# ibm-granite/dolomite-engine

Measured on AMD Instinct MI355X. Metric: tokens/sec/node GPTDolomite-3B bf16 seq4096 padding-free, higher is better.
Workload: dtype bf16; 1 GPU; gptdolomite-3b-bf16-seq4096-paddingfree-pretrain; model=GPTDolomite-3B, global_batch=16, seq_len=4096, parallelism=dp1

## Files before the change

### dolomite_engine_amd/csrc/attention.hip

```cpp

#include "common.h"

typedef __bf16 bf16x8 __attribute__((ext_vector_type(8)));
typedef float f32x4 __attribute__((ext_vector_type(4)));
typedef uint32_t u32x4 __attribute__((ext_vector_type(4)));

#define MFMA16(a, b, c) __builtin_amdgcn_mfma_f32_16x16x32_bf16((a), (b), (c), 0, 0, 0)

#define DOL_LOG2E 1.44269504088896340736f
#define DOL_LN2 0.69314718055994530942f

#define PI23(q) (((q) & ~12) | ((((q) >> 2) & 1) << 3) | ((((q) >> 3) & 1) << 2))

typedef __bf16 bf16x4 __attribute__((ext_vector_type(4)));


__device__ __forceinline__ bf16x8 lds_tr16_bfrag(const __bf16* img, int rowbase, int S, int d0, int lane) {
    const int g8 = (lane >> 4) * 8;
    const int jj = (lane >> 2) & 3;
    const int cc = (lane & 3) * 4;
    unsigned a0 = (unsigned)(size_t)(img + PI23(rowbase + g8 + jj) * S + d0 + cc);
    unsigned a1 = (unsigned)(size_t)(img + PI23(rowbase + g8 + 4 + jj) * S + d0 + cc);
    bf16x4 lo, hi;
    asm volatile(
        "ds_read_b64_tr_b16 %0, %2\n\t"
        "ds_read_b64_tr_b16 %1, %3\n\t"
        "s_waitcnt lgkmcnt(0)"
        : "=&v"(lo), "=&v"(hi)
        : "v"(a0), "v"(a1)
        : "memory");
    bf16x8 out;
#pragma unroll
    for (int t = 0; t < 4; ++t) { out[t] = lo[t]; out[4 + t] = hi[t]; }
    return out;
}


template <int OFF>
__device__ __forceinline__ void tr16_issue(unsigned a0, unsigned a1, bf16x4& lo, bf16x4& hi) {
    asm volatile(
        "ds_read_b64_tr_b16 %0, %2 offset:%c4\n\t"
        "ds_read_b64_tr_b16 %1, %3 offset:%c4"
        : "=&v"(lo), "=&v"(hi)
        : "v"(a0), "v"(a1), "i"(OFF)
        : "memory");
}

template <int N>
__device__ __forceinline__ void lgkm_wait2(bf16x4& a, bf16x4& b) {
    asm volatile("s_waitcnt lgkmcnt(%c2)" : "+v"(a), "+v"(b) : "i"(N));
}
template <int N>
__device__ __forceinline__ void lgkm_wait4(bf16x4& a, bf16x4& b, bf16x4& c, bf16x4& d) {
    asm volatile("s_waitcnt lgkmcnt(%c4)" : "+v"(a), "+v"(b), "+v"(c), "+v"(d) : "i"(N));
}
template <int N>
__device__ __forceinline__ void lgkm_wait8(bf16x4& a, bf16x4& b, bf16x4& c, bf16x4& d,
                                           bf16x4& e, bf16x4& f, bf16x4& g, bf16x4& h) {
    asm volatile("s_waitcnt lgkmcnt(%c8)"
                 : "+v"(a), "+v"(b), "+v"(c), "+v"(d), "+v"(e), "+v"(f), "+v"(g), "+v"(h)
                 : "i"(N));
}

__device__ __forceinline__ bf16x8 tr16_join8(bf16x4 lo, bf16x4 hi) {
    bf16x8 out;
#pragma unroll
    for (int t = 0; t < 4; ++t) { out[t] = lo[t]; out[4 + t] = hi[t]; }
    return out;
}

__device__ __forceinline__ bf16x8 load_bf16x8_guard(const __bf16* p, int d0, int D, bool valid) {
    const __bf16* q = (d0 < D) ? p : (p - d0);
    bool ok = valid && (d0 < D);
    bf16x8 r = *(const bf16x8*)q;
#pragma unroll
    for (int e = 0; e < 8; ++e) r[e] = ok ? r[e] : (__bf16)0.f;
    return r;
}

__device__ __forceinline__ void xcd_remap_tile_bh(int& tile, int& b, int& h) {
    const int ntile = gridDim.x, nb = gridDim.y, nh = gridDim.z;
    const int64_t nbh = (int64_t)nb * nh;
    if (nbh % 8 != 0) return;
    int64_t raw = blockIdx.x + (int64_t)ntile * (blockIdx.y + (int64_t)nb * blockIdx.z);
    int xcd = (int)(raw % 8);
    int64_t idx = raw / 8;
    int64_t pair_local = idx / ntile;
    tile = (int)(idx % ntile);
    int64_t pair = pair_local * 8 + xcd;
    b = (int)(pair % nb);
    h = (int)(pair / nb);
}

#define DOL_DROP_CQ 0x9E3779B1u
#define DOL_DROP_CK 0x85EBCA77u
#define DOL_DROP_CH 0xC2B2AE3Du
#define DOL_DROP_M1 0x7FEB352Du
#define DOL_DROP_M2 0x846CA68Bu

__device__ __forceinline__ uint32_t drop_mix32(uint32_t x) {
    x ^= x >> 16;
    x *= DOL_DROP_M1;
    x ^= x >> 15;
    x *= DOL_DROP_M2;
    x ^= x >> 16;
    return x;
}
__device__ __forceinline__ uint32_t drop_head_word(uint32_t seed_hi, uint32_t h) {
    return drop_mix32(seed_hi ^ (h * DOL_DROP_CH));
}
__device__ __forceinline__ uint32_t drop_row_word(uint32_t seed_lo, uint32_t t_q) {
    return drop_mix32(seed_lo ^ (t_q * DOL_DROP_CQ));
}
__device__ __forceinline__ uint32_t drop_col_word(uint32_t head_word, uint32_t t_k) {
    return drop_mix32(head_word ^ (t_k * DOL_DROP_CK));
}
__device__ __forceinline__ bool drop_keep_words(uint32_t rw, uint32_t cw, uint32_t thr) {
    uint32_t x = rw ^ cw;
    x ^= x >> 16;
    x *= DOL_DROP_M1;
    x ^= x >> 15;
    x *= DOL_DROP_M2;
    return x >= thr;
}
__device__ __forceinline__ bool drop_keep(uint32_t seed_lo, uint32_t seed_hi, uint32_t h,
                                          uint32_t t_q, uint32_t t_k, uint32_t thr) {
    return drop_keep_words(drop_row_word(seed_lo, t_q),
                           drop_col_word(drop_head_word(seed_hi, h), t_k), thr);
}

static inline uint32_t drop_threshold(float p_drop) {
    return (uint32_t)((double)p_drop * 4294967296.0);
}
static inline bool drop_p_valid(float p_drop) { return p_drop >= 0.f && p_drop < 1.f; }


template <int DPAD>
struct FaKvLds {
    static constexpr int S = DPAD + 16;
    static constexpr size_t image_bytes = (size_t)2 * 64 * S * sizeof(__bf16);
    static constexpr size_t bytes(bool dropout) {
        return image_bytes + (dropout ? 64 * sizeof(uint32_t) : 0);
    }
};

__device__ __forceinline__ void fa_tr16_perm_bases(const __bf16* img, int S, int lane,
                                                   unsigned& a0, unsigned& a1) {
    const int row = (lane >> 4) * 4 + ((lane >> 2) & 3);
    const int cc = (lane & 3) * 4;
    a0 = (unsigned)(size_t)(img + row * S + cc);
    a1 = (unsigned)(size_t)(img + (16 + row) * S + cc);
}

__device__ __forceinline__ float qgroup_reduce_max(float v) {
    auto a = __builtin_amdgcn_permlane16_swap(__float_as_uint(v), __float_as_uint(v), false, false);
    v = fmaxf(__uint_as_float(a[0]), __uint_as_float(a[1]));
    auto b = __builtin_amdgcn_permlane32_swap(__float_as_uint(v), __float_as_uint(v), false, false);
    return fmaxf(__uint_as_float(b[0]), __uint_as_float(b[1]));
}
__device__ __forceinline__ float qgroup_reduce_sum(float v) {
    auto a = __builtin_amdgcn_permlane16_swap(__float_as_uint(v), __float_as_uint(v), false, false);
    v = __uint_as_float(a[0]) + __uint_as_float(a[1]);
    auto b = __builtin_amdgcn_permlane32_swap(__float_as_uint(v), __float_as_uint(v), false, false);
    return __uint_as_float(b[0]) + __uint_as_float(b[1]);
}


template <int DPAD, bool DROPOUT>
__global__ void __launch_bounds__(512, 4) fa_fwd_kernel(
    const __bf16* __restrict__ q, const __bf16* __restrict__ k, const __bf16* __restrict__ v,
    __bf16* __restrict__ o, float* __restrict__ lse,
    const int32_t* __restrict__ seq_begin, const int32_t* __restrict__ seq_end,
    int H, int Hkv, int D, int G,
    int64_t q_ts, int64_t q_gs, int64_t k_ts, int64_t k_hs, int64_t v_ts, int64_t v_hs,
    int64_t o_ts, int64_t T_total, float scale,
    uint32_t seed_lo, uint32_t seed_hi, uint32_t drop_thr, float drop_rp) {
    constexpr int KCH = DPAD / 32;
    constexpr int DCH = DPAD / 16;
    constexpr int SK = FaKvLds<DPAD>::S;

    int tile_id = blockIdx.x, b = blockIdx.y, h = blockIdx.z;
    xcd_remap_tile_bh(tile_id, b, h);
    const int s0 = __builtin_amdgcn_readfirstlane(seq_begin[b]);
    const int L = __builtin_amdgcn_readfirstlane(seq_end[b]) - s0;
    const int ntile_seq = (L + 127) / 128;
    if (tile_id >= ntile_seq) return;
    const int qs = (ntile_seq - 1 - tile_id) * 128;

    const int lane = threadIdx.x & 63;
    const int wave = threadIdx.x >> 6;
    const int lr = lane & 15;
    const int lg = lane >> 4;

    extern __shared__ char smem_raw[];
    __bf16* Klds = (__bf16*)smem_raw;
    __bf16* Vlds = Klds + 64 * SK;
    uint32_t* Cw = (uint32_t*)(Vlds + 64 * SK);

    const int kvh = h / G;
    const int64_t q_hoff = (int64_t)(h / G) * q_gs + (int64_t)(h % G) * D;

    const int qrow = qs + wave * 16 + lr;
    const bool qvalid = qrow < L;
    bf16x8 qf[KCH];
#pragma unroll
    for (int kc = 0; kc < KCH; ++kc) {
        int d0 = kc * 32 + lg * 8;
        const __bf16* p = q + (int64_t)(s0 + (qvalid ? qrow : 0)) * q_ts + q_hoff + d0;
        qf[kc] = load_bf16x8_guard(p, d0, D, qvalid);
    }

    float m_run = -INFINITY, l_run = 0.f;
    f32x4 o_acc[DCH];
#pragma unroll
    for (int dc = 0; dc < DCH; ++dc) o_acc[dc] = {0.f, 0.f, 0.f, 0.f};

    uint32_t drop_rw = 0;
    uint32_t drop_hw = 0;
    if constexpr (DROPOUT) {
        drop_hw = drop_head_word(seed_hi, (uint32_t)h);
        drop_rw = drop_row_word(seed_lo, (uint32_t)(s0 + qrow));
    }

    unsigned aV0, aV1;
    fa_tr16_perm_bases(Vlds, SK, lane, aV0, aV1);

    const int kend = min(L, qs + 128);
    const int ntiles = (kend + 63) / 64;

    if (D < DPAD) {
        for (int pidx = threadIdx.x; pidx < 64 * (DPAD - D) / 8; pidx += 512) {
            int key = pidx / ((DPAD - D) / 8);
            int d0 = D + (pidx % ((DPAD - D) / 8)) * 8;
            bf16x8 z = {};
            *(bf16x8*)&Klds[key * SK + d0] = z;
            *(bf16x8*)&Vlds[key * SK + d0] = z;
        }
    }

    int st_koff[2], st_voff[2];
    int st_klds[2], st_vlds[2];
#pragma unroll
    for (int j = 0; j < 2; ++j) {
        int pidx = (int)threadIdx.x + j * 512;
        int pp = pidx < 64 * D / 8 ? pidx : 0;
        int key = pp / (D / 8);
        int d0 = (pp % (D / 8)) * 8;
        st_koff[j] = (int)(key * k_ts + kvh * k_hs) + d0;
        st_voff[j] = (int)(key * v_ts + kvh * v_hs) + d0;
        st_klds[j] = key * SK + d0;
        st_vlds[j] = key * SK + d0;
    }

    if (__builtin_amdgcn_readfirstlane(threadIdx.x) >= 256) __builtin_amdgcn_s_setprio(1);

    constexpr int PIECES = 64 * DPAD / 8;

    auto stage_direct = [&](int ks_, __bf16* Kw, __bf16* Vw) {
        if (ks_ + 64 <= kend) {
            const int64_t disp = (int64_t)(s0 + ks_);
#pragma unroll
            for (int j = 0; j < 2; ++j) {
                if ((int)threadIdx.x + j * 512 < 64 * D / 8) {
                    *(bf16x8*)&Kw[st_klds[j]] = *(const bf16x8*)(k + disp * k_ts + st_koff[j]);
                    *(bf16x8*)&Vw[st_vlds[j]] = *(const bf16x8*)(v + disp * v_ts + st_voff[j]);
                }
            }
        } else {
            for (int pidx = threadIdx.x; pidx < PIECES; pidx += 512) {
                int key = pidx / (DPAD / 8);
                int d0 = (pidx % (DPAD / 8)) * 8;
                bool kv_valid = (ks_ + key) < kend;
                const __bf16* kp = k + (int64_t)(s0 + (kv_valid ? ks_ + key : 0)) * k_ts + (int64_t)kvh * k_hs + d0;
                *(bf16x8*)&Kw[key * SK + d0] = load_bf16x8_guard(kp, d0, D, kv_valid);
                const __bf16* vp = v + (int64_t)(s0 + (kv_valid ? ks_ + key : 0)) * v_ts + (int64_t)kvh * v_hs + d0;
                *(bf16x8*)&Vw[key * SK + d0] = load_bf16x8_guard(vp, d0, D, kv_valid);
            }
        }
    };

    const float scale2 = scale * DOL_LOG2E;

    auto compute_tile = [&](const __bf16* Kb, unsigned aV0c, unsigned aV1c, int ks) {
        f32x4 sc[4];
#pragma unroll
        for (int cb = 0; cb < 4; ++cb) {
            sc[cb] = {0.f, 0.f, 0.f, 0.f};
#pragma unroll
            for (int kc = 0; kc < KCH; ++kc) {
                bf16x8 kf = *(const bf16x8*)&Kb[(cb * 16 + lr) * SK + kc * 32 + lg * 8];
                sc[cb] = MFMA16(kf, qf[kc], sc[cb]);
            }
        }

        const bool edge_tile =
            !((ks + 63 <= qs + wave * 16) && (ks + 64 <= kend) && (qs + wave * 16 + 16 <= L));
        if (__builtin_amdgcn_readfirstlane(edge_tile ? 1 : 0)) {
#pragma unroll
            for (int cb = 0; cb < 4; ++cb) {
#pragma unroll
                for (int x = 0; x < 4; ++x) {
                    const int kpos = ks + cb * 16 + lg * 4 + x;
                    if (kpos > qrow || kpos >= kend || qrow >= L) sc[cb][x] = -INFINITY;
                }
            }
        }
        float mx[4];
#pragma unroll
        for (int cb = 0; cb < 4; ++cb)
            mx[cb] = fmaxf(fmaxf(sc[cb][0], sc[cb][1]), fmaxf(sc[cb][2], sc[cb][3]));
        const float rowmax = qgroup_reduce_max(fmaxf(fmaxf(mx[0], mx[1]), fmaxf(mx[2], mx[3])));
        float mnew = fmaxf(m_run, rowmax * scale2);
        if (mnew == -INFINITY) mnew = 0.f;
        const float alpha = exp2f(m_run - mnew);
        m_run = mnew;

        bf16x8 pf[2];
        float rsum = 0.f;
#pragma unroll
        for (int cb = 0; cb < 4; ++cb) {
            u32x4 cw = {};
            if constexpr (DROPOUT) cw = *(const u32x4*)&Cw[cb * 16 + lg * 4];
#pragma unroll
            for (int x = 0; x < 4; ++x) {
                const float e = exp2f(fmaf(sc[cb][x], scale2, -mnew));
                float ek = e;
                if constexpr (DROPOUT) ek = drop_keep_words(drop_rw, cw[x], drop_thr) ? e : 0.f;
                pf[cb >> 1][(cb & 1) * 4 + x] = (__bf16)ek;
                rsum += e;
            }
        }
        l_run = l_run * alpha + rsum;
        if (!__all(alpha == 1.0f)) {
#pragma unroll
            for (int dc = 0; dc < DCH; ++dc) o_acc[dc] *= alpha;
        }

        {
            __builtin_amdgcn_sched_barrier(0);
            bf16x4 vlo[3], vhi[3];
            tr16_issue<0>(aV0c, aV1c, vlo[0], vhi[0]);
            tr16_issue<((1 / DCH) * 32 * SK + (1 % DCH) * 16) * 2>(aV0c, aV1c, vlo[1], vhi[1]);
#define FWD_PV_STEP(i)                                                                                  \
    if constexpr ((i) < 2 * DCH) {                                                                      \
        constexpr int kc2_ = (i) / DCH, dc_ = (i) % DCH;                                                \
        if constexpr ((i) + 2 < 2 * DCH) {                                                              \
            constexpr int kn_ = ((i) + 2) / DCH, dn_ = ((i) + 2) % DCH;                                 \
            tr16_issue<(kn_ * 32 * SK + dn_ * 16) * 2>(aV0c, aV1c, vlo[((i) + 2) % 3], vhi[((i) + 2) % 3]); \
            lgkm_wait2<4>(vlo[(i) % 3], vhi[(i) % 3]);                                                  \
        } else if constexpr ((i) + 1 < 2 * DCH) {                                                       \
            lgkm_wait2<2>(vlo[(i) % 3], vhi[(i) % 3]);                                                  \
        } else {                                                                                        \
            lgkm_wait2<0>(vlo[(i) % 3], vhi[(i) % 3]);                                                  \
        }                                                                                               \
        o_acc[dc_] = MFMA16(tr16_join8(vlo[(i) % 3], vhi[(i) % 3]), pf[kc2_], o_acc[dc_]);              \
    }
            FWD_PV_STEP(0) FWD_PV_STEP(1) FWD_PV_STEP(2) FWD_PV_STEP(3)
            FWD_PV_STEP(4) FWD_PV_STEP(5) FWD_PV_STEP(6) FWD_PV_STEP(7)
            FWD_PV_STEP(8) FWD_PV_STEP(9) FWD_PV_STEP(10) FWD_PV_STEP(11)
            FWD_PV_STEP(12) FWD_PV_STEP(13) FWD_PV_STEP(14) FWD_PV_STEP(15)
#undef FWD_PV_STEP
            __builtin_amdgcn_sched_barrier(0);
        }
    };

    for (int kt = 0; kt < ntiles; ++kt) {
        stage_direct(kt * 64, Klds, Vlds);
        if constexpr (DROPOUT) {
            if (__builtin_amdgcn_readfirstlane(threadIdx.x) < 64)
                Cw[lane] = drop_col_word(drop_hw, (uint32_t)(s0 + kt * 64 + lane));
        }
        __syncthreads();
        compute_tile(Klds, aV0, aV1, kt * 64);
        __syncthreads();
    }

    const float l_row = qgroup_reduce_sum(l_run);
    float inv_l = (l_row > 0.f) ? 1.f / l_row : 0.f;
    if constexpr (DROPOUT) inv_l *= drop_rp;
    if (lg == 0 && qvalid)
        lse[(int64_t)h * T_total + s0 + qrow] = (m_run + log2f(l_row)) * DOL_LN2;
    __bf16* orow = o + (int64_t)(s0 + (qvalid ? qrow : 0)) * o_ts + (int64_t)h * D;
#pragma unroll
    for (int dc = 0; dc < DCH; ++dc) {
        const int d0 = dc * 16 + lg * 4;
        bf16x4 ov;
#pragma unroll
        for (int x = 0; x < 4; ++x) ov[x] = (__bf16)(o_acc[dc][x] * inv_l);
        if (qvalid && d0 < D) *(bf16x4*)&orow[d0] = ov;
    }
}

struct FaProblem {
    dolomite_stream_t stream;
    const void *q, *k, *v;
    void* o;
    const void* dout;
    float* lse;
    const float* delta;
    void* dqkv_q;
    float *dk_acc, *dv_acc;
    const int32_t *seq_begin, *seq_end;
    int batch, max_seqlen;
    int64_t T;
    int H, Hkv, D, G;
    int64_t q_ts, q_gs, k_ts, k_hs, v_ts, v_hs, do_ts;
    float scale;
    int dtype;
    float p_drop;
    uint64_t seed;
    bool gaps;
};

static int fa_check_args(const FaProblem& p, bool fwd) {
    if (!drop_p_valid(p.p_drop)) return 9013;
    if (p.dtype != DOLOMITE_BF16) return 9010;
    if (p.D > 128) return 9011;
    if (fwd && !(p.scale > 0.f)) return 9015;
    return 0;
}

template <typename Launch>
static int fa_select_kernel(const FaProblem& p, Launch launch) {
    auto by_dpad = [&](auto drop) {
        if (p.D <= 32) return launch(std::integral_constant<int, 32>{}, drop);
        if (p.D <= 64) return launch(std::integral_constant<int, 64>{}, drop);
        if (p.D <= 96) return launch(std::integral_constant<int, 96>{}, drop);
        return launch(std::integral_constant<int, 128>{}, drop);
    };
    return p.p_drop > 0.f ? by_dpad(std::true_type{}) : by_dpad(std::false_type{});
}

static dim3 fa_grid(const FaProblem& p) { return dim3((p.max_seqlen + 127) / 128, p.batch, p.H); }

template <int DPAD, bool DROPOUT>
static int launch_fa_fwd(const FaProblem& p) {
    hipLaunchKernelGGL((fa_fwd_kernel<DPAD, DROPOUT>), fa_grid(p), dim3(512), FaKvLds<DPAD>::bytes(DROPOUT),
                       (hipStream_t)p.stream, (const __bf16*)p.q, (const __bf16*)p.k, (const __bf16*)p.v,
                       (__bf16*)p.o, p.lse, p.seq_begin, p.seq_end, p.H, p.Hkv, p.D, p.G,
                       p.q_ts, p.q_gs, p.k_ts, p.k_hs, p.v_ts, p.v_hs, (int64_t)p.H * p.D, p.T, p.scale,
                       (uint32_t)p.seed, (uint32_t)(p.seed >> 32), drop_threshold(p.p_drop),
                       1.f / (1.f - p.p_drop));
    return dol_last_error();
}

static int fa_spans_fwd_dispatch(const FaProblem& p) {
    int err = fa_check_args(p, true);
    if (err) return err;
    if (p.gaps) {
        err = dolomite_fa_zero_gap_rows(p.stream, p.o, (int64_t)p.H * p.D * (int64_t)sizeof(__bf16),
                                        p.seq_begin, p.seq_end, p.batch, p.T);
        if (err) return err;
        if (p.batch == 0 || p.max_seqlen <= 0) return 0;
    }
    return fa_select_kernel(p, [&](auto dpad, auto drop) {
        return launch_fa_fwd<decltype(dpad)::value, decltype(drop)::value>(p);
    });
}

extern "C" int dolomite_fa_varlen_fwd(dolomite_stream_t stream,
                                      const void* q, const void* k, const void* v,
                                      void* o, float* lse,
                                      const int32_t* cu_seqlens, int batch, int max_seqlen, int64_t T,
                                      int H, int Hkv, int D, int G,
                                      int64_t q_tstride, int64_t q_gstride,
                                      int64_t k_tstride, int64_t k_hstride,
                                      int64_t v_tstride, int64_t v_hstride,
                                      float scale, int dtype) {
    return fa_spans_fwd_dispatch({stream, q, k, v, o, nullptr, lse, nullptr, nullptr, nullptr, nullptr,
                                  cu_seqlens, cu_seqlens + 1, batch, max_seqlen, T, H, Hkv, D, G,
                                  q_tstride, q_gstride, k_tstride, k_hstride, v_tstride, v_hstride, 0,
                                  scale, dtype, 0.f, 0, false});
}

extern "C" int dolomite_fa_varlen_fwd_dropout(dolomite_stream_t stream,
                                              const void* q, const void* k, const void* v,
                                              void* o, float* lse,
                                              const int32_t* cu_seqlens, int batch, int max_seqlen, int64_t T,
                                              int H, int Hkv, int D, int G,
                                              int64_t q_tstride, int64_t q_gstride,
                                              int64_t k_tstride, int64_t k_hstride,
                                              int64_t v_tstride, int64_t v_hstride,
                                              float scale, int dtype, float p_drop, uint64_t seed) {
    return fa_spans_fwd_dispatch({stream, q, k, v, o, nullptr, lse, nullptr, nullptr, nullptr, nullptr,
                                  cu_seqlens, cu_seqlens + 1, batch, max_seqlen, T, H, Hkv, D, G,
                                  q_tstride, q_gstride, k_tstride, k_hstride, v_tstride, v_hstride, 0,
                                  scale, dtype, p_drop, seed, false});
}


template <typename T>
__global__ void __launch_bounds__(256) fa_bwd_preprocess_kernel(
    const T* __restrict__ o, const T* __restrict__ dout, float* __restrict__ delta,
    int64_t T_total, int H, int D, int64_t o_ts, int64_t do_ts) {
    int64_t row = ((int64_t)blockIdx.x * 4) + (threadIdx.x >> 6);
    int lane = threadIdx.x & 63;
    if (row >= T_total * H) return;
    int64_t t = row / H;
    int h = (int)(row % H);
    const T* op = o + t * o_ts + (int64_t)h * D;
    const T* dp = dout + t * do_ts + (int64_t)h * D;
    float acc = 0.f;
    for (int d = lane * 2; d + 1 < D; d += 128) {
        float o0[2], d0[2];
        VecIO<T, 2>::load(op + d, o0);
        VecIO<T, 2>::load(dp + d, d0);
        acc += o0[0] * d0[0] + o0[1] * d0[1];
    }
    if (D & 1) {
        int d = D - 1;
        if (lane == 0) acc += load_as_f32(op + d) * load_as_f32(dp + d);
    }
    acc = wave_reduce_sum(acc);
    if (lane == 0) delta[(int64_t)h * T_total + t] = acc;
}

__global__ void __launch_bounds__(256) fa_bwd_preprocess_tiled(
    const __bf16* __restrict__ o, const __bf16* __restrict__ dout, float* __restrict__ delta,
    int64_t T_total, int H, int D, int TOK) {
    extern __shared__ float part[];
    const int64_t hd = (int64_t)H * D;
    const int64_t base = (int64_t)blockIdx.x * TOK * hd;
    const int64_t total = T_total * hd;
    const int np = (int)(TOK * hd / 8);
#pragma unroll 4
    for (int p = threadIdx.x; p < np; p += 256) {
        int64_t flat = base + (int64_t)p * 8;
        float acc = 0.f;
        if (flat + 8 <= total) {
            bf16x8 ov = *(const bf16x8*)(o + flat);
            bf16x8 dv = *(const bf16x8*)(dout + flat);
#pragma unroll
            for (int e = 0; e < 8; ++e) acc += (float)ov[e] * (float)dv[e];
        }
        part[p] = acc;
    }
    __syncthreads();
    const int slots = TOK * H;
    const int dp8 = D / 8;
    for (int s = threadIdx.x; s < slots; s += 256) {
        float a = 0.f;
        const float* ps = &part[s * dp8];
        for (int i = 0; i < dp8; ++i) a += ps[i];
        int tl = s / H, h = s - tl * H;
        int64_t t = (int64_t)blockIdx.x * TOK + tl;
        if (t < T_total) delta[(int64_t)h * T_total + t] = a;
    }
}

extern "C" int dolomite_fa_bwd_preprocess(dolomite_stream_t stream,
                                          const void* o, const void* dout, float* delta,
                                          int64_t T, int H, int D,
                                          int64_t o_tstride, int64_t do_tstride, int dtype) {
    const int64_t hd = (int64_t)H * D;
    int TOK = 16;
    while (TOK > 1 && TOK * hd * 4 / 8 > 65536) TOK /= 2;
    if (dtype == DOLOMITE_BF16 && D % 8 == 0 && o_tstride == hd && do_tstride == hd && T > 0 &&
        TOK * hd * 4 / 8 <= 65536) {
        dim3 grid((uint32_t)((T + TOK - 1) / TOK)), block(256);
        size_t shmem = (size_t)(TOK * hd / 8) * sizeof(float);
        hipLaunchKernelGGL((fa_bwd_preprocess_tiled), grid, block, shmem, (hipStream_t)stream,
                           (const __bf16*)o, (const __bf16*)dout, delta, T, H, D, TOK);
        return dol_last_error();
    }
    int64_t rows = T * H;
    dim3 grid((uint32_t)((rows + 3) / 4)), block(256);
    if (dtype == DOLOMITE_BF16)
        hipLaunchKernelGGL((fa_bwd_preprocess_kernel<uint16_t>), grid, block, 0, (hipStream_t)stream,
                           (const uint16_t*)o, (const uint16_t*)dout, delta, T, H, D, o_tstride, do_tstride);
    else
        hipLaunchKernelGGL((fa_bwd_preprocess_kernel<float>), grid, block, 0, (hipStream_t)stream,
                           (const float*)o, (const float*)dout, delta, T, H, D, o_tstride, do_tstride);
    return dol_last_error();
}




__device__ __forceinline__ float dkv_exp2(float x) { return __builtin_amdgcn_exp2f(x); }

template <int DPAD>
struct FaDkvLds {
    static constexpr int S = FaKvLds<DPAD>::S;
    static constexpr size_t image_bytes = (size_t)2 * 64 * S * sizeof(__bf16);
    static constexpr size_t bytes(bool dropout) {
        return image_bytes + 2 * 64 * sizeof(float) + (dropout ? 64 * sizeof(uint32_t) : 0);
    }
};

template <int DPAD, bool DROPOUT>
__global__ void __launch_bounds__(512, DPAD <= 96 ? 4 : 2) fa_bwd_dkv_kernel(
    const __bf16* __restrict__ q, const __bf16* __restrict__ k, const __bf16* __restrict__ v,
    const __bf16* __restrict__ dout, const float* __restrict__ lse, const float* __restrict__ delta,
    float* __restrict__ dk_acc, float* __restrict__ dv_acc,
    const int32_t* __restrict__ seq_begin, const int32_t* __restrict__ seq_end,
    int H, int Hkv, int D, int G,
    int64_t q_ts, int64_t q_gs, int64_t k_ts, int64_t k_hs, int64_t v_ts, int64_t v_hs,
    int64_t do_ts, int64_t T_total, float scale,
    uint32_t seed_lo, uint32_t seed_hi, uint32_t drop_thr, float drop_rp) {
    constexpr int KCH = DPAD / 32;
    constexpr int DCH = DPAD / 16;

    int tile_id = blockIdx.x, b = blockIdx.y, h = blockIdx.z;
    xcd_remap_tile_bh(tile_id, b, h);
    const int kvh = h / G;
    const int s0 = __builtin_amdgcn_readfirstlane(seq_begin[b]);
    const int L = __builtin_amdgcn_readfirstlane(seq_end[b]) - s0;
    const int ks = tile_id * 128;
    if (ks >= L) return;

    const int lane = threadIdx.x & 63;
    const int wave = threadIdx.x >> 6;
    const int lr = lane & 15;
    const int lg = lane >> 4;

    constexpr int SQ = FaDkvLds<DPAD>::S;
    extern __shared__ char smem_raw[];
    __bf16* Qlds = (__bf16*)smem_raw;
    __bf16* dOl = Qlds + 64 * SQ;
    float* Lsel = (float*)(dOl + 64 * SQ);
    float* NDel = Lsel + 64;
    uint32_t* Rw = (uint32_t*)(NDel + 64);

    const int kend = min(L, ks + 128);

    const int krow = ks + wave * 16 + lr;
    const bool kvalid = krow < kend;
    bf16x8 kfr[KCH], vfr[KCH];
#pragma unroll
    for (int kc = 0; kc < KCH; ++kc) {
        int d0 = kc * 32 + lg * 8;
        const __bf16* kp = k + (int64_t)(s0 + (kvalid ? krow : 0)) * k_ts + (int64_t)kvh * k_hs + d0;
        kfr[kc] = load_bf16x8_guard(kp, d0, D, kvalid);
        const __bf16* vp = v + (int64_t)(s0 + (kvalid ? krow : 0)) * v_ts + (int64_t)kvh * v_hs + d0;
        vfr[kc] = load_bf16x8_guard(vp, d0, D, kvalid);
    }

    f32x4 dvr[DCH], dkr[DCH];
#pragma unroll
    for (int dc = 0; dc < DCH; ++dc) {
        dvr[dc] = {0.f, 0.f, 0.f, 0.f};
        dkr[dc] = {0.f, 0.f, 0.f, 0.f};
    }

    uint32_t drop_cw = 0;
    if constexpr (DROPOUT)
        drop_cw = drop_col_word(drop_head_word(seed_hi, (uint32_t)h), (uint32_t)(s0 + krow));

    unsigned aQ0, aQ1;
    fa_tr16_perm_bases(Qlds, SQ, lane, aQ0, aQ1);
    constexpr int DO_IMM = 64 * SQ * 2;
    static_assert(DO_IMM + 32 * SQ * 2 + DPAD * 2 < 65536, "ds offset range");
    const float scale2 = scale * DOL_LOG2E;

    if (__builtin_amdgcn_readfirstlane(threadIdx.x) >= 256) __builtin_amdgcn_s_setprio(1);

    const int qt0 = ks / 64;
    const int nqt = (L + 63) / 64;
    const int64_t q_hoff = (int64_t)(h / G) * q_gs + (int64_t)(h % G) * D;
    const int64_t do_hoff = (int64_t)h * D;

    if (D < DPAD) {
        for (int pidx = threadIdx.x; pidx < 64 * (DPAD - D) / 8; pidx += 512) {
            int qq = pidx / ((DPAD - D) / 8);
            int d0 = D + (pidx % ((DPAD - D) / 8)) * 8;
            bf16x8 z = {};
            *(bf16x8*)&Qlds[qq * SQ + d0] = z;
            *(bf16x8*)&dOl[qq * SQ + d0] = z;
        }
    }

    auto dkv_chunk = [&](auto cc, const int qs, const int full) {
        constexpr int c = decltype(cc)::value;
        bf16x8 pf, dsf;
#pragma unroll
        for (int hb = 0; hb < 2; ++hb) {
            const int cb = 2 * c + hb;
            f32x4 st = {0.f, 0.f, 0.f, 0.f};
            f32x4 dpt = {0.f, 0.f, 0.f, 0.f};
            if constexpr (!DROPOUT) dpt = *(const f32x4*)&NDel[cb * 16 + lg * 4];
#pragma unroll
            for (int kc = 0; kc < KCH; ++kc) {
                int d0 = kc * 32 + lg * 8;
                bf16x8 qa = *(const bf16x8*)&Qlds[(cb * 16 + lr) * SQ + d0];
                st = MFMA16(qa, kfr[kc], st);
                bf16x8 da = *(const bf16x8*)&dOl[(cb * 16 + lr) * SQ + d0];
                dpt = MFMA16(da, vfr[kc], dpt);
            }
            const f32x4 ls = *(const f32x4*)&Lsel[cb * 16 + lg * 4];
            u32x4 rw = {};
            f32x4 nd = {};
            if constexpr (DROPOUT) {
                rw = *(const u32x4*)&Rw[cb * 16 + lg * 4];
                nd = *(const f32x4*)&NDel[cb * 16 + lg * 4];
            }
            if (full) {
#pragma unroll
                for (int x = 0; x < 4; ++x) {
                    float pv = dkv_exp2(fmaf(st[x], scale2, -ls[x]));
                    if constexpr (DROPOUT) {
                        const bool keep = drop_keep_words(rw[x], drop_cw, drop_thr);
                        pf[hb * 4 + x] = (__bf16)(keep ? pv : 0.f);
                        dsf[hb * 4 + x] = (__bf16)(pv * fmaf(keep ? dpt[x] : 0.f, drop_rp, nd[x]));
                    } else {
                        pf[hb * 4 + x] = (__bf16)pv;
                        dsf[hb * 4 + x] = (__bf16)(pv * dpt[x]);
                    }
                }
            } else {
#pragma unroll
                for (int x = 0; x < 4; ++x) {
                    const int qpos = qs + cb * 16 + lg * 4 + x;
                    const bool ok = kvalid && qpos < L && krow <= qpos;
                    float pv = ok ? dkv_exp2(fmaf(st[x], scale2, -ls[x])) : 0.f;
                    if constexpr (DROPOUT) {
                        const bool keep = drop_keep_words(rw[x], drop_cw, drop_thr);
                        float ds = ok ? pv * fmaf(keep ? dpt[x] : 0.f, drop_rp, nd[x]) : 0.f;
                        pf[hb * 4 + x] = (__bf16)(keep ? pv : 0.f);
                        dsf[hb * 4 + x] = (__bf16)ds;
                    } else {
                        float ds = ok ? pv * dpt[x] : 0.f;
                        pf[hb * 4 + x] = (__bf16)pv;
                        dsf[hb * 4 + x] = (__bf16)ds;
                    }
                }
            }
        }

        __builtin_amdgcn_sched_barrier(0);
        constexpr int CB = c * 32 * SQ * 2;
        bf16x4 alo[3], ahi[3];
        tr16_issue<CB + DO_IMM>(aQ0, aQ1, alo[0], ahi[0]);
        static_assert(DCH >= 2, "fragment 1 is the dO image's second 16-col block");
        tr16_issue<CB + DO_IMM + 32>(aQ0, aQ1, alo[1], ahi[1]);
#define DKV_STEP(i)                                                                                     \
    if constexpr ((i) < 2 * DCH) {                                                                      \
        constexpr int im_ = (i) / DCH, dc_ = (i) % DCH;                                                 \
        if constexpr ((i) + 2 < 2 * DCH) {                                                              \
            constexpr int in_ = ((i) + 2) / DCH, dn_ = ((i) + 2) % DCH;                                 \
            tr16_issue<CB + (in_ ? 0 : DO_IMM) + dn_ * 32>(aQ0, aQ1, alo[((i) + 2) % 3], ahi[((i) + 2) % 3]); \
            lgkm_wait2<4>(alo[(i) % 3], ahi[(i) % 3]);                                                  \
        } else if constexpr ((i) + 1 < 2 * DCH) {                                                       \
            lgkm_wait2<2>(alo[(i) % 3], ahi[(i) % 3]);                                                  \
        } else {                                                                                        \
            lgkm_wait2<0>(alo[(i) % 3], ahi[(i) % 3]);                                                  \
        }                                                                                               \
        if constexpr (im_ == 0)                                                                         \
            dvr[dc_] = MFMA16(tr16_join8(alo[(i) % 3], ahi[(i) % 3]), pf, dvr[dc_]);                    \
        else                                                                                            \
            dkr[dc_] = MFMA16(tr16_join8(alo[(i) % 3], ahi[(i) % 3]), dsf, dkr[dc_]);                   \
    }
        DKV_STEP(0) DKV_STEP(1) DKV_STEP(2) DKV_STEP(3)
        DKV_STEP(4) DKV_STEP(5) DKV_STEP(6) DKV_STEP(7)
        DKV_STEP(8) DKV_STEP(9) DKV_STEP(10) DKV_STEP(11)
        DKV_STEP(12) DKV_STEP(13) DKV_STEP(14) DKV_STEP(15)
#undef DKV_STEP
        __builtin_amdgcn_sched_barrier(0);
    };

    const unsigned st_magic = (1u << 22) / (unsigned)(D / 8) + 1;
    for (int qt = qt0; qt < nqt; ++qt) {
        const int qs = qt * 64;
        __syncthreads();
        {
            const int pieces = 64 * DPAD / 8;
            if (qs + 64 <= L) {
                for (int pidx = threadIdx.x; pidx < 64 * D / 8; pidx += 512) {
                    int qq = (int)(((unsigned)pidx * st_magic) >> 22);
                    int d0 = (pidx - qq * (D / 8)) * 8;
                    *(bf16x8*)&Qlds[qq * SQ + d0] =
                        *(const bf16x8*)(q + (int64_t)(s0 + qs + qq) * q_ts + q_hoff + d0);
                    *(bf16x8*)&dOl[qq * SQ + d0] =
                        *(const bf16x8*)(dout + (int64_t)(s0 + qs + qq) * do_ts + do_hoff + d0);
                }
            } else {
                for (int pidx = threadIdx.x; pidx < pieces; pidx += 512) {
                    int qq = pidx / (DPAD / 8);
                    int d0 = (pidx % (DPAD / 8)) * 8;
                    bool valid = (qs + qq) < L;
                    const __bf16* qp = q + (int64_t)(s0 + (valid ? qs + qq : 0)) * q_ts + q_hoff + d0;
                    *(bf16x8*)&Qlds[qq * SQ + d0] = load_bf16x8_guard(qp, d0, D, valid);
                    const __bf16* dp = dout + (int64_t)(s0 + (valid ? qs + qq : 0)) * do_ts + do_hoff + d0;
                    *(bf16x8*)&dOl[qq * SQ + d0] = load_bf16x8_guard(dp, d0, D, valid);
                }
            }
            const int swave = __builtin_amdgcn_readfirstlane(wave);
            const bool sok = qs + lane < L;
            const int64_t sidx = (int64_t)h * T_total + s0 + (sok ? qs + lane : 0);
            if (swave == 0) {
                Lsel[lane] = sok ? lse[sidx] * DOL_LOG2E : 0.f;
            } else if (swave == 1) {
                NDel[lane] = sok ? -delta[sidx] : 0.f;
            } else if (swave == 2) {
                if constexpr (DROPOUT) Rw[lane] = drop_row_word(seed_lo, (uint32_t)(s0 + qs + lane));
            }
        }
        __syncthreads();

        const bool full_tile = (ks + wave * 16 + 16 <= qs + 1) && (ks + wave * 16 + 16 <= kend) && (qs + 64 <= L);
        const int full = __builtin_amdgcn_readfirstlane(full_tile ? 1 : 0);
        dkv_chunk(std::integral_constant<int, 0>{}, qs, full);
        dkv_chunk(std::integral_constant<int, 1>{}, qs, full);
    }

    const int64_t rowoff = ((int64_t)(s0 + (kvalid ? krow : 0)) * H + h) * D;
#pragma unroll
    for (int dc = 0; dc < DCH; ++dc) {
        const int d0 = dc * 16 + lg * 4;
        if (kvalid && d0 < D) {
            f32x4 dkv4 = dkr[dc] * scale;
            __builtin_nontemporal_store(dkv4, (f32x4*)&dk_acc[rowoff + d0]);
            f32x4 dvv4 = dvr[dc];
            if constexpr (DROPOUT) dvv4 *= drop_rp;
            __builtin_nontemporal_store(dvv4, (f32x4*)&dv_acc[rowoff + d0]);
        }
    }
}

template <int DPAD, bool DROPOUT>
__global__ void __launch_bounds__(512, (DROPOUT && DPAD > 96) ? 2 : 4) fa_bwd_dq_kernel(
    const __bf16* __restrict__ q, const __bf16* __restrict__ k, const __bf16* __restrict__ v,
    const __bf16* __restrict__ dout, const float* __restrict__ lse, const float* __restrict__ delta,
    __bf16* __restrict__ dqkv_q,
    const int32_t* __restrict__ seq_begin, const int32_t* __restrict__ seq_end,
    int H, int Hkv, int D, int G,
    int64_t q_ts, int64_t q_gs, int64_t k_ts, int64_t k_hs, int64_t v_ts, int64_t v_hs,
    int64_t do_ts, int64_t T_total, float scale,
    uint32_t seed_lo, uint32_t seed_hi, uint32_t drop_thr, float drop_rp) {
    constexpr int KCH = DPAD / 32;
    constexpr int DCH = DPAD / 16;

    int tile_id = blockIdx.x, b = blockIdx.y, h = blockIdx.z;
    xcd_remap_tile_bh(tile_id, b, h);
    const int kvh = h / G;
    const int s0 = __builtin_amdgcn_readfirstlane(seq_begin[b]);
    const int L = __builtin_amdgcn_readfirstlane(seq_end[b]) - s0;
    const int ntile_seq = (L + 127) / 128;
    if (tile_id >= ntile_seq) return;
    const int qs = (ntile_seq - 1 - tile_id) * 128;

    const int lane = threadIdx.x & 63;
    const int wave = threadIdx.x >> 6;
    const int lr = lane & 15;
    const int lg = lane >> 4;

    constexpr int SQ = FaKvLds<DPAD>::S;
    extern __shared__ char smem_raw[];
    __bf16* Klds = (__bf16*)smem_raw;
    __bf16* Vlds = Klds + 64 * SQ;
    uint32_t* Cw = (uint32_t*)(Vlds + 64 * SQ);

    const int64_t q_hoff = (int64_t)(h / G) * q_gs + (int64_t)(h % G) * D;
    const int64_t do_hoff = (int64_t)h * D;

    unsigned aK0, aK1;
    fa_tr16_perm_bases(Klds, SQ, lane, aK0, aK1);

    const int qrow = qs + wave * 16 + lr;
    const bool qvalid = qrow < L;
    bf16x8 qfr[KCH], dfr[KCH];
#pragma unroll
    for (int kc = 0; kc < KCH; ++kc) {
        int d0 = kc * 32 + lg * 8;
        const __bf16* qp = q + (int64_t)(s0 + (qvalid ? qrow : 0)) * q_ts + q_hoff + d0;
        qfr[kc] = load_bf16x8_guard(qp, d0, D, qvalid);
        const __bf16* dp = dout + (int64_t)(s0 + (qvalid ? qrow : 0)) * do_ts + do_hoff + d0;
        dfr[kc] = load_bf16x8_guard(dp, d0, D, qvalid);
    }

    const float lsev = qvalid ? lse[(int64_t)h * T_total + s0 + qrow] * DOL_LOG2E : 0.f;
    const float delv = qvalid ? delta[(int64_t)h * T_total + s0 + qrow] : 0.f;
    const float scale2 = scale * DOL_LOG2E;

    f32x4 dq[DCH];
#pragma unroll
    for (int dc = 0; dc < DCH; ++dc) dq[dc] = {0.f, 0.f, 0.f, 0.f};

    uint32_t drop_rw = 0;
    uint32_t drop_hw = 0;
    if constexpr (DROPOUT) {
        drop_hw = drop_head_word(seed_hi, (uint32_t)h);
        drop_rw = drop_row_word(seed_lo, (uint32_t)(s0 + qrow));
    }

    if (D < DPAD) {
        for (int pidx = threadIdx.x; pidx < 64 * (DPAD - D) / 8; pidx += 512) {
            int key = pidx / ((DPAD - D) / 8);
            int d0 = D + (pidx % ((DPAD - D) / 8)) * 8;
            bf16x8 z = {};
            *(bf16x8*)&Klds[key * SQ + d0] = z;
            *(bf16x8*)&Vlds[key * SQ + d0] = z;
        }
    }

    int st_koff[2], st_voff[2];
    int st_klds[2], st_vlds[2];
#pragma unroll
    for (int j = 0; j < 2; ++j) {
        int pidx = (int)threadIdx.x + j * 512;
        int pp = pidx < 64 * D / 8 ? pidx : 0;
        int key = pp / (D / 8);
        int d0 = (pp % (D / 8)) * 8;
        st_koff[j] = (int)(key * k_ts + kvh * k_hs) + d0;
        st_voff[j] = (int)(key * v_ts + kvh * v_hs) + d0;
        st_klds[j] = key * SQ + d0;
        st_vlds[j] = key * SQ + d0;
    }

    const int kend_total = min(L, qs + 128);
    const int nkt = (kend_total + 63) / 64;

    if (__builtin_amdgcn_readfirstlane(threadIdx.x) >= 256) __builtin_amdgcn_s_setprio(1);

    for (int kt = 0; kt < nkt; ++kt) {
        const int ks = kt * 64;
        __syncthreads();
        {
            const int pieces = 64 * DPAD / 8;
            if (ks + 64 <= kend_total) {
                const int64_t disp = (int64_t)(s0 + ks);
#pragma unroll
                for (int j = 0; j < 2; ++j) {
                    if ((int)threadIdx.x + j * 512 < 64 * D / 8) {
                        *(bf16x8*)&Klds[st_klds[j]] = *(const bf16x8*)(k + disp * k_ts + st_koff[j]);
                        *(bf16x8*)&Vlds[st_vlds[j]] = *(const bf16x8*)(v + disp * v_ts + st_voff[j]);
                    }
                }
            } else {
                for (int pidx = threadIdx.x; pidx < pieces; pidx += 512) {
                    int key = pidx / (DPAD / 8);
                    int d0 = (pidx % (DPAD / 8)) * 8;
                    bool valid = (ks + key) < kend_total;
                    const __bf16* kp = k + (int64_t)(s0 + (valid ? ks + key : 0)) * k_ts + (int64_t)kvh * k_hs + d0;
                    *(bf16x8*)&Klds[key * SQ + d0] = load_bf16x8_guard(kp, d0, D, valid);
                    const __bf16* vp = v + (int64_t)(s0 + (valid ? ks + key : 0)) * v_ts + (int64_t)kvh * v_hs + d0;
                    *(bf16x8*)&Vlds[key * SQ + d0] = load_bf16x8_guard(vp, d0, D, valid);
                }
            }
            if constexpr (DROPOUT) {
                if (__builtin_amdgcn_readfirstlane(threadIdx.x) < 64)
                    Cw[lane] = drop_col_word(drop_hw, (uint32_t)(s0 + ks + lane));
            }
        }
        __syncthreads();

        const bool full_tile = (ks + 64 <= qs + wave * 16 + 1) && (ks + 64 <= kend_total) && (qs + wave * 16 + 16 <= L);
        bf16x8 dsf[2];
#pragma unroll
        for (int cb = 0; cb < 4; ++cb) {
            f32x4 sc = {0.f, 0.f, 0.f, 0.f};
            f32x4 dp = {0.f, 0.f, 0.f, 0.f};
#pragma unroll
            for (int kc = 0; kc < KCH; ++kc) {
                int d0 = kc * 32 + lg * 8;
                bf16x8 kb = *(const bf16x8*)&Klds[(cb * 16 + lr) * SQ + d0];
                sc = MFMA16(kb, qfr[kc], sc);
                bf16x8 vb = *(const bf16x8*)&Vlds[(cb * 16 + lr) * SQ + d0];
                dp = MFMA16(vb, dfr[kc], dp);
            }
            u32x4 cw = {};
            if constexpr (DROPOUT) cw = *(const u32x4*)&Cw[cb * 16 + lg * 4];
            if (__builtin_amdgcn_readfirstlane(full_tile ? 1 : 0)) {
#pragma unroll
                for (int x = 0; x < 4; ++x) {
                    float pv = exp2f(fmaf(sc[x], scale2, -lsev));
                    float dpm = dp[x];
                    if constexpr (DROPOUT)
                        dpm = drop_keep_words(drop_rw, cw[x], drop_thr) ? dp[x] * drop_rp : 0.f;
                    dsf[cb >> 1][(cb & 1) * 4 + x] = (__bf16)(pv * (dpm - delv) * scale);
                }
            } else {
#pragma unroll
                for (int x = 0; x < 4; ++x) {
                    const int kpos = ks + cb * 16 + lg * 4 + x;
                    bool ok = qvalid && kpos < kend_total && kpos <= qrow;
                    float pv = ok ? exp2f(fmaf(sc[x], scale2, -lsev)) : 0.f;
                    float dpm = dp[x];
                    if constexpr (DROPOUT)
                        dpm = drop_keep_words(drop_rw, cw[x], drop_thr) ? dp[x] * drop_rp : 0.f;
                    float ds = ok ? pv * (dpm - delv) * scale : 0.f;
                    dsf[cb >> 1][(cb & 1) * 4 + x] = (__bf16)ds;
                }
            }
        }

        {
            __builtin_amdgcn_sched_barrier(0);
            bf16x4 klo[4], khi[4];
            tr16_issue<0>(aK0, aK1, klo[0], khi[0]);
            tr16_issue<((1 / DCH) * 32 * SQ + (1 % DCH) * 16) * 2>(aK0, aK1, klo[1], khi[1]);
            tr16_issue<((2 / DCH) * 32 * SQ + (2 % DCH) * 16) * 2>(aK0, aK1, klo[2], khi[2]);
#define DQ_STEP(i)                                                                                      \
    if constexpr ((i) < 2 * DCH) {                                                                      \
        constexpr int kc2_ = (i) / DCH, dc_ = (i) % DCH;                                                \
        if constexpr ((i) + 3 < 2 * DCH) {                                                              \
            constexpr int kn_ = ((i) + 3) / DCH, dn_ = ((i) + 3) % DCH;                                 \
            tr16_issue<(kn_ * 32 * SQ + dn_ * 16) * 2>(aK0, aK1, klo[((i) + 3) % 4], khi[((i) + 3) % 4]); \
            lgkm_wait2<6>(klo[(i) % 4], khi[(i) % 4]);                                                  \
        } else if constexpr ((i) + 2 < 2 * DCH) {                                                       \
            lgkm_wait2<4>(klo[(i) % 4], khi[(i) % 4]);                                                  \
        } else if constexpr ((i) + 1 < 2 * DCH) {                                                       \
            lgkm_wait2<2>(klo[(i) % 4], khi[(i) % 4]);                                                  \
        } else {                                                                                        \
            lgkm_wait2<0>(klo[(i) % 4], khi[(i) % 4]);                                                  \
        }                                                                                               \
        dq[dc_] = MFMA16(tr16_join8(klo[(i) % 4], khi[(i) % 4]), dsf[kc2_], dq[dc_]);                   \
    }
            DQ_STEP(0) DQ_STEP(1) DQ_STEP(2) DQ_STEP(3)
            DQ_STEP(4) DQ_STEP(5) DQ_STEP(6) DQ_STEP(7)
            DQ_STEP(8) DQ_STEP(9) DQ_STEP(10) DQ_STEP(11)
            DQ_STEP(12) DQ_STEP(13) DQ_STEP(14) DQ_STEP(15)
#undef DQ_STEP
            __builtin_amdgcn_sched_barrier(0);
        }
    }

    __bf16* dqrow = dqkv_q + (int64_t)(s0 + (qvalid ? qrow : 0)) * q_ts + q_hoff;
#pragma unroll
    for (int dc = 0; dc < DCH; ++dc) {
        const int d0 = dc * 16 + lg * 4;
        bf16x4 dv;
#pragma unroll
        for (int x = 0; x < 4; ++x) dv[x] = (__bf16)dq[dc][x];
        if (qvalid && d0 < D) *(bf16x4*)&dqrow[d0] = dv;
    }
}

template <int DPAD, bool DROPOUT>
static int launch_fa_bwd(const FaProblem& p) {
    const dim3 grid = fa_grid(p), block(512);
    const hipStream_t stream = (hipStream_t)p.stream;
    const __bf16 *q = (const __bf16*)p.q, *k = (const __bf16*)p.k, *v = (const __bf16*)p.v;
    const __bf16* dout = (const __bf16*)p.dout;
    const uint32_t seed_lo = (uint32_t)p.seed, seed_hi = (uint32_t)(p.seed >> 32);
    const uint32_t thr = drop_threshold(p.p_drop);
    const float rp = 1.f / (1.f - p.p_drop);
    hipLaunchKernelGGL((fa_bwd_dkv_kernel<DPAD, DROPOUT>), grid, block, FaDkvLds<DPAD>::bytes(DROPOUT), stream,
                       q, k, v, dout, p.lse, p.delta, p.dk_acc, p.dv_acc, p.seq_begin, p.seq_end,
                       p.H, p.Hkv, p.D, p.G, p.q_ts, p.q_gs, p.k_ts, p.k_hs, p.v_ts, p.v_hs, p.do_ts,
                       p.T, p.scale, seed_lo, seed_hi, thr, rp);
    int err = dol_last_error();
    if (err) return err;
    hipLaunchKernelGGL((fa_bwd_dq_kernel<DPAD, DROPOUT>), grid, block, FaKvLds<DPAD>::bytes(DROPOUT), stream,
                       q, k, v, dout, p.lse, p.delta, (__bf16*)p.dqkv_q, p.seq_begin, p.seq_end,
                       p.H, p.Hkv, p.D, p.G, p.q_ts, p.q_gs, p.k_ts, p.k_hs, p.v_ts, p.v_hs, p.do_ts,
                       p.T, p.scale, seed_lo, seed_hi, thr, rp);
    return dol_last_error();
}

static int fa_spans_bwd_dispatch(const FaProblem& p) {
    int err = fa_check_args(p, false);
    if (err) return err;
    if (p.gaps && (p.batch == 0 || p.max_seqlen <= 0)) return 0;
    return fa_select_kernel(p, [&](auto dpad, auto drop) {
        return launch_fa_bwd<decltype(dpad)::value, decltype(drop)::value>(p);
    });
}

extern "C" int dolomite_fa_varlen_bwd(dolomite_stream_t stream,
                                      const void* q, const void* k, const void* v,
                                      const void* dout, const float* lse,
                                      const float* delta, void* dqkv_q, float* dk_acc, float* dv_acc,
                                      const int32_t* cu_seqlens, int batch, int max_seqlen, int64_t T,
                                      int H, int Hkv, int D, int G,
                                      int64_t q_tstride, int64_t q_gstride,
                                      int64_t k_tstride, int64_t k_hstride,
                                      int64_t v_tstride, int64_t v_hstride,
                                      int64_t do_tstride,
                                      float scale, int dtype) {
    return fa_spans_bwd_dispatch({stream, q, k, v, nullptr, dout, const_cast<float*>(lse), delta, dqkv_q,
                                  dk_acc, dv_acc, cu_seqlens, cu_seqlens + 1, batch, max_seqlen, T,
                                  H, Hkv, D, G, q_tstride, q_gstride, k_tstride, k_hstride,
                                  v_tstride, v_hstride, do_tstride, scale, dtype, 0.f, 0, false});
}

extern "C" int dolomite_fa_varlen_bwd_dropout(dolomite_stream_t stream,
                                              const void* q, const void* k, const void* v,
                                              const void* dout, const float* lse,
                                              const float* delta, void* dqkv_q, float* dk_acc, float* dv_acc,
                                              const int32_t* cu_seqlens, int batch, int max_seqlen, int64_t T,
                                              int H, int Hkv, int D, int G,
                                              int64_t q_tstride, int64_t q_gstride,
                                              int64_t k_tstride, int64_t k_hstride,
                                              int64_t v_tstride, int64_t v_hstride,
                                              int64_t do_tstride,
                                              float scale, int dtype, float p_drop, uint64_t seed) {
    return fa_spans_bwd_dispatch({stream, q, k, v, nullptr, dout, const_cast<float*>(lse), delta, dqkv_q,
                                  dk_acc, dv_acc, cu_seqlens, cu_seqlens + 1, batch, max_seqlen, T,
                                  H, Hkv, D, G, q_tstride, q_gstride, k_tstride, k_hstride,
                                  v_tstride, v_hstride, do_tstride, scale, dtype, p_drop, seed, false});
}


__global__ void __launch_bounds__(256) fa_zero_gap_rows_kernel(
    uint4* __restrict__ buf, int64_t row_vec,
    const int32_t* __restrict__ seq_begin, const int32_t* __restrict__ seq_end,
    int batch, int64_t T) {
    const int g = blockIdx.y;
    int64_t lo = g == 0 ? 0 : (int64_t)seq_end[g - 1];
    int64_t hi = g == batch ? T : (int64_t)seq_begin[g];
    lo = lo < 0 ? 0 : lo;
    hi = hi > T ? T : hi;
    if (hi <= lo) return;
    const int64_t first = lo * row_vec, last = hi * row_vec;
    const uint4 z = {0u, 0u, 0u, 0u};
    for (int64_t i = first + (int64_t)blockIdx.x * 256 + threadIdx.x; i < last;
         i += (int64_t)gridDim.x * 256)
        buf[i] = z;
}

extern "C" int dolomite_fa_zero_gap_rows(dolomite_stream_t stream, void* buf, int64_t row_bytes,
                                         const int32_t* seq_begin, const int32_t* seq_end,
                                         int batch, int64_t T) {
    if (row_bytes <= 0 || row_bytes % 16 != 0) return 9016;
    if (batch < 0 || T < 0 || batch >= 65535) return 9014;
    if (T == 0) return 0;
    const int64_t vec_per_gap = (T * (row_bytes / 16) + batch) / (batch + 1);
    int64_t chunks = (vec_per_gap + 1023) / 1024;
    chunks = chunks < 1 ? 1 : (chunks > 1024 ? 1024 : chunks);
    hipLaunchKernelGGL(fa_zero_gap_rows_kernel, dim3((uint32_t)chunks, (uint32_t)(batch + 1)),
                       dim3(256), 0, (hipStream_t)stream, (uint4*)buf, row_bytes / 16,
                       seq_begin, seq_end, batch, T);
    return dol_last_error();
}

extern "C" int dolomite_fa_spans_fwd(dolomite_stream_t stream,
                                     const void* q, const void* k, const void* v,
                                     void* o, float* lse,
                                     const int32_t* seq_begin, const int32_t* seq_end,
                                     int batch, int max_seqlen, int64_t T,
                                     int H, int Hkv, int D, int G,
                                     int64_t q_tstride, int64_t q_gstride,
                                     int64_t k_tstride, int64_t k_hstride,
                                     int64_t v_tstride, int64_t v_hstride,
                                     float scale, int dtype, float p_drop, uint64_t seed) {
    return fa_spans_fwd_dispatch({stream, q, k, v, o, nullptr, lse, nullptr, nullptr, nullptr, nullptr,
                                  seq_begin, seq_end, batch, max_seqlen, T, H, Hkv, D, G,
                                  q_tstride, q_gstride, k_tstride, k_hstride, v_tstride, v_hstride, 0,
                                  scale, dtype, p_drop, seed, true});
}

extern "C" int dolomite_fa_spans_bwd(dolomite_stream_t stream,
                                     const void* q, const void* k, const void* v,
                                     const void* dout, const float* lse,
                                     const float* delta, void* dqkv_q, float* dk_acc, float* dv_acc,
                                     const int32_t* seq_begin, const int32_t* seq_end,
                                     int batch, int max_seqlen, int64_t T,
                                     int H, int Hkv, int D, int G,
                                     int64_t q_tstride, int64_t q_gstride,
                                     int64_t k_tstride, int64_t k_hstride,
                                     int64_t v_tstride, int64_t v_hstride,
                                     int64_t do_tstride,
                                     float scale, int dtype, float p_drop, uint64_t seed) {
    return fa_spans_bwd_dispatch({stream, q, k, v, nullptr, dout, const_cast<float*>(lse), delta, dqkv_q,
                                  dk_acc, dv_acc, seq_begin, seq_end, batch, max_seqlen, T,
                                  H, Hkv, D, G, q_tstride, q_gstride, k_tstride, k_hstride,
                                  v_tstride, v_hstride, do_tstride, scale, dtype, p_drop, seed, true});
}

__global__ void __launch_bounds__(256) fa_dropout_mask_probe_kernel(
    uint8_t* __restrict__ out, uint32_t seed_lo, uint32_t seed_hi, uint32_t thr,
    int64_t total, int64_t tq0, int nq, int64_t tk0, int nk) {
    const int64_t idx = (int64_t)blockIdx.x * 256 + threadIdx.x;
    if (idx >= total) return;
    const int j = (int)(idx % nk);
    const int64_t hi = idx / nk;
    const int i = (int)(hi % nq);
    const uint32_t h = (uint32_t)(hi / nq);
    out[idx] = drop_keep(seed_lo, seed_hi, h, (uint32_t)(tq0 + i), (uint32_t)(tk0 + j), thr) ? 1 : 0;
}

extern "C" int dolomite_fa_dropout_mask_probe(dolomite_stream_t stream, uint8_t* out,
                                              uint64_t seed, float p_drop, int H,
                                              int64_t tq0, int nq, int64_t tk0, int nk) {
    if (!drop_p_valid(p_drop)) return 9013;
    if (H < 0 || nq < 0 || nk < 0) return 9014;
    const int64_t total = (int64_t)H * nq * nk;
    if (total == 0) return 0;
    const int64_t nblocks = (total + 255) / 256;
    if (nblocks > 0x7fffffff) return 9014;
    hipLaunchKernelGGL(fa_dropout_mask_probe_kernel, dim3((uint32_t)nblocks), dim3(256), 0,
                       (hipStream_t)stream, out, (uint32_t)seed, (uint32_t)(seed >> 32),
                       drop_threshold(p_drop), total, tq0, nq, tk0, nk);
    return dol_last_error();
}


template <typename T>
__global__ void __launch_bounds__(256) fa_grad_finalize_kernel(
    const float* __restrict__ dk_acc, const float* __restrict__ dv_acc,
    T* __restrict__ dqkv, int64_t total_kv,
    int Hkv, int D, int G, int64_t row_ts, int64_t k_off, int64_t kv_hs, int64_t v_off) {
    int64_t quad = (int64_t)blockIdx.x * blockDim.x + threadIdx.x;
    int64_t total_q4 = total_kv / 4;
    bool is_v = quad >= total_q4;
    if (is_v) quad -= total_q4;
    if (quad >= total_q4) return;
    int64_t kidx = quad * 4;
    int64_t t = kidx / ((int64_t)Hkv * D);
    int rem = (int)(kidx % ((int64_t)Hkv * D));
    int j = rem / D;
    int d = rem % D;
    const float* src = is_v ? dv_acc : dk_acc;
    int64_t base = ((t * Hkv + j) * (int64_t)G) * D + d;
    f4_t acc = {0.f, 0.f, 0.f, 0.f};
    for (int g = 0; g < G; ++g) {
        f4_t v4 = __builtin_nontemporal_load((const f4_t*)&src[base + (int64_t)g * D]);
        acc += v4;
    }
    T* out = &dqkv[t * row_ts + (is_v ? v_off : k_off) + (int64_t)j * kv_hs + d];
#pragma unroll
    for (int e = 0; e < 4; ++e) store_from_f32(out + e, acc[e]);
}

extern "C" int dolomite_fa_grad_finalize(dolomite_stream_t stream,
                                         const float* dk_acc, const float* dv_acc,
                                         void* dqkv, int64_t T, int Hkv, int D, int G,
                                         int64_t row_tstride,
                                         int64_t k_off, int64_t kv_hstride, int64_t v_off, int dtype) {
    int64_t total_kv = T * (int64_t)Hkv * D;
    if (D % 4 != 0) return 9012;
    int64_t total = 2 * (total_kv / 4);
    if (total == 0) return 0;
    dim3 grid((uint32_t)((total + 255) / 256)), block(256);
    if (dtype == DOLOMITE_BF16)
        hipLaunchKernelGGL((fa_grad_finalize_kernel<uint16_t>), grid, block, 0, (hipStream_t)stream,
                           dk_acc, dv_acc, (uint16_t*)dqkv, total_kv,
                           Hkv, D, G, row_tstride, k_off, kv_hstride, v_off);
    else
        hipLaunchKernelGGL((fa_grad_finalize_kernel<float>), grid, block, 0, (hipStream_t)stream,
                           dk_acc, dv_acc, (float*)dqkv, total_kv,
                           Hkv, D, G, row_tstride, k_off, kv_hstride, v_off);
    return dol_last_error();
}


typedef __bf16 bf16x4p __attribute__((ext_vector_type(4)));
__global__ void __launch_bounds__(64) tr16_probe_kernel(float* out) {
    __shared__ __bf16 s[256];
    const int lane = threadIdx.x & 63;
    for (int i = threadIdx.x; i < 256; i += 64) s[i] = (__bf16)(float)i;
    __syncthreads();
    const unsigned base = (unsigned)(size_t)(__bf16*)s;
    unsigned addrs[3] = {
        base + (unsigned)((lane >> 4) * 128),
        base + (unsigned)(lane * 8),
        base + (unsigned)(((lane & 15) * 2) + ((lane >> 4) * 128)),
    };
#pragma unroll
    for (int v = 0; v < 3; ++v) {
        bf16x4p r;
        asm volatile("ds_read_b64_tr_b16 %0, %1\n\ts_waitcnt lgkmcnt(0)"
                     : "=v"(r)
                     : "v"(addrs[v])
                     : "memory");
#pragma unroll
        for (int j = 0; j < 4; ++j) out[(v * 64 + lane) * 4 + j] = (float)r[j];
    }
}

extern "C" int dolomite_tr16_probe(dolomite_stream_t stream, float* out) {
    hipLaunchKernelGGL(tr16_probe_kernel, dim3(1), dim3(64), 0, (hipStream_t)stream, out);
    return dol_last_error();
}

__global__ void __launch_bounds__(64) tr16_bfrag_probe_kernel(
    const __bf16* src, float* out, int cols, int S, int rowbase, int d0) {
    extern __shared__ char smem_raw[];
    __bf16* img = (__bf16*)smem_raw;
    const int lane = threadIdx.x & 63;
    for (int i = threadIdx.x; i < 64 * (cols / 8); i += 64) {
        int row = i / (cols / 8), c8 = (i % (cols / 8)) * 8;
        *(bf16x8*)&img[PI23(row) * S + c8] = *(const bf16x8*)&src[row * cols + c8];
    }
    __syncthreads();
    bf16x8 f = lds_tr16_bfrag(img, rowbase, S, d0, lane);
#pragma unroll
    for (int e = 0; e < 8; ++e) out[lane * 8 + e] = (float)f[e];
}

extern "C" int dolomite_tr16_bfrag_probe(dolomite_stream_t stream, const void* src, float* out,
                                         int cols, int S, int rowbase, int d0) {
    size_t shmem = (size_t)64 * S * sizeof(__bf16);
    hipLaunchKernelGGL(tr16_bfrag_probe_kernel, dim3(1), dim3(64), shmem, (hipStream_t)stream,
                       (const __bf16*)src, out, cols, S, rowbase, d0);
    return dol_last_error();
}

__global__ void __launch_bounds__(64) mfma_probe_kernel(const __bf16* A, const __bf16* B, float* C) {
    int lane = threadIdx.x & 63;
    int lr = lane & 15, lg = lane >> 4;
    bf16x8 a, b;
#pragma unroll
    for (int e = 0; e < 8; ++e) {
        a[e] = A[lr * 32 + lg * 8 + e];
        b[e] = B[(lg * 8 + e) * 16 + lr];
    }
    f32x4 c = {0.f, 0.f, 0.f, 0.f};
    c = MFMA16(a, b, c);
#pragma unroll
    for (int r = 0; r < 4; ++r) C[(lg * 4 + r) * 16 + lr] = c[r];
}

extern "C" int dolomite_mfma_probe(dolomite_stream_t stream, const void* A, const void* B, float* C) {
    hipLaunchKernelGGL(mfma_probe_kernel, dim3(1), dim3(64), 0, (hipStream_t)stream,
                       (const __bf16*)A, (const __bf16*)B, C);
    return dol_last_error();
}
```

### dolomite_engine_amd/ops/hip.py

```python

import ctypes
from pathlib import Path

import torch

_SO_PATH = Path(__file__).resolve().parent.parent / "libdolomite_hip.so"
_ABI_VERSION = 2

_lib = None

F32 = 0
BF16 = 1

_c = ctypes
_i32 = _c.c_int32
_i64 = _c.c_int64
_u64 = _c.c_uint64
_f32 = _c.c_float
_p = _c.c_void_p


_SIGNATURES = {
    "dolomite_hip_abi_version": ([], _i32),
    "dolomite_rmsnorm_fwd": ([_p, _p, _p, _p, _p, _p, _p, _i64, _i64, _f32, _i32], _i32),
    "dolomite_rmsnorm_bwd_nblocks": ([_i64], _i32),
    "dolomite_rmsnorm_bwd": ([_p, _p, _p, _p, _p, _p, _p, _p, _i64, _i64, _i32], _i32),
    "dolomite_layernorm_fwd": ([_p, _p, _p, _p, _p, _p, _p, _p, _p, _i64, _i64, _f32, _i32], _i32),
    "dolomite_layernorm_bwd": ([_p, _p, _p, _p, _p, _p, _p, _p, _p, _i64, _i64, _i32], _i32),
    "dolomite_reduce_partials": ([_p, _p, _p, _i64, _i64], _i32),
    "dolomite_rope_qkv": ([_p, _p, _p, _p, _p, _i64, _i64, _i32, _i32, _i32, _i32, _i64, _i64, _i64, _i32, _i32, _i32], _i32),
    "dolomite_fa_bwd_preprocess": ([_p, _p, _p, _p, _i64, _i32, _i32, _i64, _i64, _i32], _i32),
    "dolomite_fa_zero_gap_rows": ([_p, _p, _i64, _p, _p, _i32, _i64], _i32),
    "dolomite_fa_dropout_mask_probe": ([_p, _p, _u64, _f32, _i32, _i64, _i32, _i64, _i32], _i32),
    "dolomite_kv_cache_append": (
        [_p, _p, _p, _p, _p, _p, _p, _i32, _i32, _i32, _i32, _i32,
         _i64, _i64, _i64, _i64, _i64, _i64, _i64, _i32],
        _i32,
    ),
    "dolomite_fa_decode_scratch_floats": ([_i32, _i32, _i32, _i32], _i64),
    "dolomite_fa_decode": (
        [_p, _p, _p, _p, _p, _p, _p, _i32, _i32, _i32, _i32, _i32, _i32, _i32,
         _i64, _i64, _i64, _i64, _i64, _i64, _i64, _i64, _f32, _i32],
        _i32,
    ),
    "dolomite_fa_grad_finalize": ([_p, _p, _p, _p, _i64, _i32, _i32, _i32, _i64, _i64, _i64, _i64, _i32], _i32),
    "dolomite_ce_fwd": ([_p, _p, _p, _p, _p, _i64, _i64, _i64, _i32, _i32], _i32),
    "dolomite_ce_bwd": ([_p, _p, _p, _p, _p, _p, _i64, _i64, _i64, _i32, _i32], _i32),
    "dolomite_adamw_step": ([_p, _p, _p, _p, _i32, _p, _p, _i64, _f32, _f32, _f32, _f32, _f32, _i32, _p], _i32),
    "dolomite_sqsum": ([_p, _p, _i64, _p, _p, _i32], _i32),
    "dolomite_moe_rows_combine": ([_p, _p, _p, _p, _i64, _i32, _i32, _i32], _i32),
    "dolomite_scale_inplace": ([_p, _p, _i64, _f32, _i32], _i32),
    "dolomite_moe_gemm_fwd": ([_p, _p, _p, _p, _p, _p, _i32, _i32, _i32, _i32, _i32], _i32),
    "dolomite_moe_gemm_dgrad": ([_p, _p, _p, _p, _p, _i32, _i32, _i32, _i32, _i32], _i32),
    "dolomite_moe_gemm_wgrad": ([_p, _p, _p, _p, _p, _i32, _i32, _i32, _i32], _i32),
    "dolomite_mfma_probe": ([_p, _p, _p, _p], _i32),
    "dolomite_tr16_probe": ([_p, _p], _i32),
    "dolomite_tr16_bfrag_probe": ([_p, _p, _p, _i32, _i32, _i32, _i32], _i32),
    "dolomite_build_sample_idx_i32": ([_p, _p, _i32, _i32, _i64, _p, _i64], _i32),
    "dolomite_build_sample_idx_i64": ([_p, _p, _i32, _i32, _i64, _p, _i64], _i32),
    "dolomite_build_blending_indices": ([_p, _p, _p, _i32, _i64], _i32),
}


def _fa_signature(bwd: bool, spans: bool, dropout: bool):
    head = [_p, _p, _p, _p]
    bufs = [_p] * (6 if bwd else 2)
    bounds = [_p] * (2 if spans else 1)
    dims = [_i32, _i32, _i64, _i32, _i32, _i32, _i32]
    strides = [_i64] * (7 if bwd else 6)
    tail = [_f32, _i32] + ([_f32, _u64] if dropout else [])
    return head + bufs + bounds + dims + strides + tail, _i32


_SIGNATURES.update({
    "dolomite_fa_varlen_fwd": _fa_signature(bwd=False, spans=False, dropout=False),
    "dolomite_fa_varlen_bwd": _fa_signature(bwd=True, spans=False, dropout=False),
    "dolomite_fa_varlen_fwd_dropout": _fa_signature(bwd=False, spans=False, dropout=True),
    "dolomite_fa_varlen_bwd_dropout": _fa_signature(bwd=True, spans=False, dropout=True),
    "dolomite_fa_spans_fwd": _fa_signature(bwd=False, spans=True, dropout=True),
    "dolomite_fa_spans_bwd": _fa_signature(bwd=True, spans=True, dropout=True),
})


def so_path() -> Path:
    return _SO_PATH


def is_available() -> bool:
    return _SO_PATH.exists()


def lib() -> ctypes.CDLL:
    global _lib
    if _lib is None:
        if not _SO_PATH.exists():
            raise RuntimeError(
                f"dolomite HIP extension not found at {_SO_PATH}. The GPU hot path "
                "requires it — build with `python -m dolomite_engine_amd.csrc.build` "
                "(there is no eager fallback on GPU)."
            )
        l = ctypes.CDLL(str(_SO_PATH))
        for name, (argtypes, restype) in _SIGNATURES.items():
            fn = getattr(l, name)
            fn.argtypes = argtypes
            fn.restype = restype
        ver = l.dolomite_hip_abi_version()
        if ver != _ABI_VERSION:
            raise RuntimeError(f"dolomite_hip ABI mismatch: built {ver}, expected {_ABI_VERSION}")
        _lib = l
    return _lib


def stream() -> ctypes.c_void_p:
    return ctypes.c_void_p(torch.cuda.current_stream().cuda_stream)


def check(ret: int, what: str) -> None:
    if ret != 0:
        raise RuntimeError(f"dolomite_hip {what} failed with code {ret}")


def ptr(t: torch.Tensor | None, offset_elems: int = 0) -> ctypes.c_void_p:
    if t is None:
        return ctypes.c_void_p(0)
    return ctypes.c_void_p(t.data_ptr() + offset_elems * t.element_size())


def dt(t: torch.Tensor) -> int:
    if t.dtype == torch.bfloat16:
        return BF16
    if t.dtype == torch.float32:
        return F32
    raise TypeError(f"dolomite_hip ops support fp32/bf16, got {t.dtype}")



_PROF: dict | None = None


def enable_profiling() -> None:
    global _PROF
    _PROF = {}


def disable_profiling() -> None:
    global _PROF
    _PROF = None


class _Region:
    __slots__ = ("name", "start")

    def __init__(self, name):
        self.name = name

    def __enter__(self):
        if _PROF is not None:
            self.start = torch.cuda.Event(enable_timing=True)
            self.start.record()
        return self

    def __exit__(self, *a):
        if _PROF is not None:
            stop = torch.cuda.Event(enable_timing=True)
            stop.record()
            _PROF.setdefault(self.name, []).append((self.start, stop))
        return False


def prof(name: str) -> _Region:
    return _Region(name)


def collect_profile() -> dict:
    if _PROF is None:
        return {}
    torch.cuda.synchronize()
    out = {}
    for name, pairs in _PROF.items():
        total = sum(s.elapsed_time(e) for s, e in pairs)
        out[name] = {"count": len(pairs), "total_ms": total, "avg_ms": total / len(pairs)}
    return out
```

### include/dolomite_hip.h

```cpp

#ifndef DOLOMITE_HIP_H
#define DOLOMITE_HIP_H

#include <stdint.h>

#ifdef __cplusplus
extern "C" {
#endif

typedef void* dolomite_stream_t;

enum dolomite_dtype { DOLOMITE_F32 = 0, DOLOMITE_BF16 = 1 };

int dolomite_hip_abi_version(void);

int dolomite_rmsnorm_fwd(dolomite_stream_t stream,
                         const void* x, const void* res_in, const void* w,
                         void* y, void* res_out, float* rstd,
                         int64_t T, int64_t H, float eps, int dtype);

int dolomite_rmsnorm_bwd_nblocks(int64_t T);
int dolomite_rmsnorm_bwd(dolomite_stream_t stream,
                         const void* dy, const void* s, const void* w,
                         const float* rstd, void* dx, float* dw_partial,
                         const void* dres_in, int64_t T, int64_t H, int dtype);

int dolomite_layernorm_fwd(dolomite_stream_t stream,
                           const void* x, const void* res_in, const void* w, const void* b,
                           void* y, void* res_out, float* mean, float* rstd,
                           int64_t T, int64_t H, float eps, int dtype);
int dolomite_layernorm_bwd(dolomite_stream_t stream,
                           const void* dy, const void* s, const void* w,
                           const float* mean, const float* rstd,
                           void* dx, float* dwdb_partial,
                           const void* dres_in, int64_t T, int64_t H, int dtype);

int dolomite_reduce_partials(dolomite_stream_t stream,
                             const float* partial, float* out,
                             int64_t nblocks, int64_t H);

int dolomite_rope_qkv(dolomite_stream_t stream,
                      const void* qkv_in, void* qkv_out,
                      const float* cos_t, const float* sin_t,
                      int64_t T, int64_t row_len,
                      int H, int Hkv, int D, int G,
                      int64_t q_gstride, int64_t k_off, int64_t kv_hstride,
                      int dir, int rotate_v_copy, int dtype);

int dolomite_fa_varlen_fwd(dolomite_stream_t stream,
                           const void* q, const void* k, const void* v,
                           void* o, float* lse,
                           const int32_t* cu_seqlens, int batch, int max_seqlen, int64_t T,
                           int H, int Hkv, int D, int G,
                           int64_t q_tstride, int64_t q_gstride,
                           int64_t k_tstride, int64_t k_hstride,
                           int64_t v_tstride, int64_t v_hstride,
                           float scale, int dtype);

int dolomite_fa_bwd_preprocess(dolomite_stream_t stream,
                               const void* o, const void* dout, float* delta,
                               int64_t T, int H, int D,
                               int64_t o_tstride, int64_t do_tstride, int dtype);
int dolomite_fa_varlen_bwd(dolomite_stream_t stream,
                           const void* q, const void* k, const void* v,
                           const void* dout, const float* lse,
                           const float* delta, void* dqkv_q, float* dk_acc, float* dv_acc,
                           const int32_t* cu_seqlens, int batch, int max_seqlen, int64_t T,
                           int H, int Hkv, int D, int G,
                           int64_t q_tstride, int64_t q_gstride,
                           int64_t k_tstride, int64_t k_hstride,
                           int64_t v_tstride, int64_t v_hstride,
                           int64_t do_tstride,
                           float scale, int dtype);
int dolomite_fa_grad_finalize(dolomite_stream_t stream,
                              const float* dk_acc, const float* dv_acc,
                              void* dqkv, int64_t T, int Hkv, int D, int G,
                              int64_t row_tstride,
                              int64_t k_off, int64_t kv_hstride, int64_t v_off, int dtype);

int dolomite_fa_varlen_fwd_dropout(dolomite_stream_t stream,
                                   const void* q, const void* k, const void* v,
                                   void* o, float* lse,
                                   const int32_t* cu_seqlens, int batch, int max_seqlen, int64_t T,
                                   int H, int Hkv, int D, int G,
                                   int64_t q_tstride, int64_t q_gstride,
                                   int64_t k_tstride, int64_t k_hstride,
                                   int64_t v_tstride, int64_t v_hstride,
                                   float scale, int dtype, float p_drop, uint64_t seed);
int dolomite_fa_varlen_bwd_dropout(dolomite_stream_t stream,
                                   const void* q, const void* k, const void* v,
                                   const void* dout, const float* lse,
                                   const float* delta, void* dqkv_q, float* dk_acc, float* dv_acc,
                                   const int32_t* cu_seqlens, int batch, int max_seqlen, int64_t T,
                                   int H, int Hkv, int D, int G,
                                   int64_t q_tstride, int64_t q_gstride,
                                   int64_t k_tstride, int64_t k_hstride,
                                   int64_t v_tstride, int64_t v_hstride,
                                   int64_t do_tstride,
                                   float scale, int dtype, float p_drop, uint64_t seed);

int dolomite_fa_spans_fwd(dolomite_stream_t stream,
                          const void* q, const void* k, const void* v,
                          void* o, float* lse,
                          const int32_t* seq_begin, const int32_t* seq_end,
                          int batch, int max_seqlen, int64_t T,
                          int H, int Hkv, int D, int G,
                          int64_t q_tstride, int64_t q_gstride,
                          int64_t k_tstride, int64_t k_hstride,
                          int64_t v_tstride, int64_t v_hstride,
                          float scale, int dtype, float p_drop, uint64_t seed);
int dolomite_fa_spans_bwd(dolomite_stream_t stream,
                          const void* q, const void* k, const void* v,
                          const void* dout, const float* lse,
                          const float* delta, void* dqkv_q, float* dk_acc, float* dv_acc,
                          const int32_t* seq_begin, const int32_t* seq_end,
                          int batch, int max_seqlen, int64_t T,
                          int H, int Hkv, int D, int G,
                          int64_t q_tstride, int64_t q_gstride,
                          int64_t k_tstride, int64_t k_hstride,
                          int64_t v_tstride, int64_t v_hstride,
                          int64_t do_tstride,
                          float scale, int dtype, float p_drop, uint64_t seed);
int dolomite_fa_zero_gap_rows(dolomite_stream_t stream, void* buf, int64_t row_bytes,
                              const int32_t* seq_begin, const int32_t* seq_end,
                              int batch, int64_t T);

int dolomite_fa_dropout_mask_probe(dolomite_stream_t stream, uint8_t* out,
                                   uint64_t seed, float p_drop, int H,
                                   int64_t tq0, int nq, int64_t tk0, int nk);

int dolomite_kv_cache_append(dolomite_stream_t stream, const void* qkv,
                             const int32_t* src_begin, const int32_t* src_end,
                             const int32_t* dst_pos, void* k_cache, void* v_cache,
                             int batch, int max_rows, int Hkv, int D, int S_cap,
                             int64_t row_tstride, int64_t k_off, int64_t v_off, int64_t kv_hstride,
                             int64_t cache_bstride, int64_t cache_tstride, int64_t cache_hstride,
                             int dtype);

int64_t dolomite_fa_decode_scratch_floats(int batch, int H, int D, int nsplit);
int dolomite_fa_decode(dolomite_stream_t stream,
                       const void* q, const void* k_cache, const void* v_cache, void* o,
                       float* scratch, const int32_t* cache_len,
                       int batch, int H, int Hkv, int D, int G,
                       int max_len, int nsplit,
                       int64_t q_tstride, int64_t q_gstride,
                       int64_t k_bstride, int64_t k_tstride, int64_t k_hstride,
                       int64_t v_bstride, int64_t v_tstride, int64_t v_hstride,
                       float scale, int dtype);

int dolomite_mfma_probe(dolomite_stream_t stream,
                        const void* A, const void* B, float* C);

int dolomite_ce_fwd(dolomite_stream_t stream,
                    const void* logits, const int64_t* labels,
                    float* row_loss, float* lse,
                    int64_t T, int64_t V, int64_t row_stride,
                    int ignore_index, int dtype);
int dolomite_ce_bwd(dolomite_stream_t stream,
                    const void* logits, const int64_t* labels, const float* lse,
                    void* dlogits, const float* grad_scale_dev,
                    int64_t T, int64_t V, int64_t row_stride,
                    int ignore_index, int dtype);

int dolomite_adamw_step(dolomite_stream_t stream,
                        float* master, void* param_out_bf16,
                        const void* grad, int grad_dtype,
                        float* m, float* v,
                        int64_t n, float lr, float beta1, float beta2,
                        float eps, float weight_decay, int step,
                        const float* gscale);

int dolomite_scale_inplace(dolomite_stream_t stream, void* buf, int64_t n,
                           float scale, int dtype);

int dolomite_moe_rows_combine(dolomite_stream_t stream, const void* h,
                              const int32_t* inv, void* out,
                              int64_t T, int K, int k_top, int dtype);

int dolomite_sqsum(dolomite_stream_t stream, const void* x, int64_t n,
                   float* partials, float* out, int dtype);

int dolomite_moe_gemm_fwd(dolomite_stream_t stream, const void* x, const void* w,
                          const void* bias, void* y, const int32_t* offsets,
                          int E, int max_rows, int N, int K, int dtype);
int dolomite_moe_gemm_dgrad(dolomite_stream_t stream, const void* dy, const void* w,
                            void* dx, const int32_t* offsets,
                            int E, int max_rows, int N, int K, int dtype);
int dolomite_moe_gemm_wgrad(dolomite_stream_t stream, const void* dy, const void* x,
                            void* dw, const int32_t* offsets,
                            int E, int N, int K, int dtype);

int dolomite_build_sample_idx_i32(const int32_t* sizes, const int32_t* doc_idx,
                                  int32_t seq_length, int32_t num_epochs,
                                  int64_t tokens_per_epoch, int32_t* sample_idx,
                                  int64_t num_samples);
int dolomite_build_sample_idx_i64(const int32_t* sizes, const int32_t* doc_idx,
                                  int32_t seq_length, int32_t num_epochs,
                                  int64_t tokens_per_epoch, int64_t* sample_idx,
                                  int64_t num_samples);
int dolomite_build_blending_indices(int16_t* dataset_index, int64_t* dataset_sample_index,
                                    const double* weights, int32_t num_datasets,
                                    int64_t size);

#ifdef __cplusplus
}
#endif

#endif
```

### tools_kernel_micro.py

```python
import math
import statistics
import sys
import time

import torch

from dolomite_engine_amd.ops import functional as Fx
from dolomite_engine_amd.ops import hip

T, H, Hkv, D = 65536, 32, 1, 80
dev = "cuda"
torch.manual_seed(0)
PEAK = 6.3e3


def timed(fn, k=30):
    for _ in range(5):
        fn()
    torch.cuda.synchronize()
    e0 = torch.cuda.Event(enable_timing=True)
    e1 = torch.cuda.Event(enable_timing=True)
    e0.record()
    for _ in range(k):
        fn()
    e1.record()
    torch.cuda.synchronize()
    return e0.elapsed_time(e1) / k


def timed_median(fn, n=20, warm=5):
    for _ in range(warm):
        fn()
    torch.cuda.synchronize()
    ts = []
    for _ in range(n):
        e0 = torch.cuda.Event(enable_timing=True)
        e1 = torch.cuda.Event(enable_timing=True)
        e0.record()
        fn()
        e1.record()
        torch.cuda.synchronize()
        ts.append(e0.elapsed_time(e1))
    return statistics.median(ts), min(ts), max(ts)


COPY_CEILING = 6.29e3


def decode_case():
    import torch.nn.functional as F

    from dolomite_engine_amd.ops.functional import QKVLayout

    shapes = [
        ("3B attention shape", "mqa", 32, 1, 80, 16, 4096),
        ("bandwidth-sized   ", "gqa", 32, 8, 128, 32, 8192),
    ]
    for name, head_type, H, Hkv, D, B, n in shapes:
        lo = QKVLayout.make(H, Hkv, D, head_type)
        qkv = (torch.randn(B, lo.row_len, device=dev) * 0.5).to(torch.bfloat16)
        k = (torch.randn(B, n, Hkv, D, device=dev) * 0.5).to(torch.bfloat16)
        v = (torch.randn(B, n, Hkv, D, device=dev) * 0.5).to(torch.bfloat16)
        lens = torch.full((B,), n, dtype=torch.int32, device=dev)
        scale = 1.0 / math.sqrt(D)
        gb = 2 * B * n * Hkv * D * 2 / 1e9
        qh = torch.stack(
            [qkv[:, (h // lo.G) * lo.q_gstride + (h % lo.G) * D:][:, :D] for h in range(H)], dim=1
        ).unsqueeze(2).contiguous()
        kh, vh = k.permute(0, 2, 1, 3), v.permute(0, 2, 1, 3)
        print(f"--- {name}: {head_type} H={H} Hkv={Hkv} D={D} B={B} cache={n}  K/V {gb * 1e3:.1f} MB ---")
        with torch.no_grad():
            ref = F.scaled_dot_product_attention(qh, kh, vh, scale=scale, enable_gqa=True)
            ref = ref.squeeze(2).reshape(B, H * D).float()
            auto = Fx.decode_num_splits(B, lo, n)
            for ns in sorted({1, auto, 2 * auto, 4 * auto}):
                fn = lambda: Fx.decode_attention(qkv, lo, k, v, lens, scale, n, num_splits=ns)
                err = (fn().float() - ref).abs().max().item()
                med, lo_t, hi_t = timed_median(fn)
                tag = " (default)" if ns == auto else ""
                print(f"decode nsplit={ns:3d}{tag:10s}: {med * 1e3:8.1f} us [{lo_t * 1e3:.1f}..{hi_t * 1e3:.1f}]  "
                      f"{gb / med * 1e3:6.0f} GB/s ({gb / med * 1e3 / COPY_CEILING * 100:4.1f}% of the copy ceiling)  "
                      f"max|o - sdpa| {err:.2e}")
            med, lo_t, hi_t = timed_median(
                lambda: F.scaled_dot_product_attention(qh, kh, vh, scale=scale, enable_gqa=True))
            print(f"torch SDPA (enable_gqa)    : {med * 1e3:8.1f} us [{lo_t * 1e3:.1f}..{hi_t * 1e3:.1f}]  "
                  f"{gb / med * 1e3:6.0f} GB/s ({gb / med * 1e3 / COPY_CEILING * 100:4.1f}% of the copy ceiling)")
        del qkv, k, v, kh, vh

    import bench
    from dolomite_engine_amd.hf_models import GPTDolomiteConfig, GPTDolomiteForCausalLM

    cfg = GPTDolomiteConfig(**bench.MODEL_350M)
    cfg._attn_implementation = "flash_attention_2"
    model = GPTDolomiteForCausalLM(cfg).to(torch.bfloat16).to(dev).eval()
    for B, S in ((1, 512), (16, 512)):
        ids = torch.randint(0, cfg.vocab_size, (B, S), device=dev)
        model.generate(ids, max_new_tokens=8)
        torch.cuda.synchronize()
        ts = []
        for _ in range(3):
            t0 = time.perf_counter()
            out = model.generate(ids, max_new_tokens=128)
            torch.cuda.synchronize()
            ts.append(time.perf_counter() - t0)
        t = statistics.median(ts)
        print(f"generate 350M greedy B={B:2d} prompt={S} +128 tokens: {t * 1e3:7.1f} ms "
              f"(prefill included)  {B * 128 / t:7.0f} tokens/s  {128 / t:6.1f} steps/s")
        assert out.shape == (B, S + 128)


if len(sys.argv) > 1 and sys.argv[1] == "decode":
    decode_case()
    sys.exit(0)

o = torch.randn(T, H * D, dtype=torch.bfloat16, device=dev)
do = torch.randn(T, H * D, dtype=torch.bfloat16, device=dev)
delta = torch.empty(H, T, dtype=torch.float32, device=dev)


def pre():
    hip.check(
        hip.lib().dolomite_fa_bwd_preprocess(
            hip.stream(), hip.ptr(o), hip.ptr(do), hip.ptr(delta), T, H, D, H * D, H * D, hip.BF16
        ),
        "pre",
    )


ms = timed(pre)
gb = (2 * T * H * D * 2 + H * T * 4) / 1e9
print(f"preprocess : {ms:6.3f} ms  {gb/ms*1e3:6.0f} GB/s ({gb/ms*1e3/PEAK*100:4.1f}% of peak)")

ref = (o.view(T, H, D).float() * do.view(T, H, D).float()).sum(-1).t().contiguous()
err = (delta - ref).abs().max().item()
print(f"             max|err| vs torch fp32: {err:.3e}")

G = H // Hkv
dk_acc = torch.randn(T, H, D, dtype=torch.float32, device=dev)
dv_acc = torch.randn(T, H, D, dtype=torch.float32, device=dev)
row_len = (H + 2 * Hkv) * D
dqkv = torch.empty(T, row_len, dtype=torch.bfloat16, device=dev)


def fin():
    hip.check(
        hip.lib().dolomite_fa_grad_finalize(
            hip.stream(), hip.ptr(dk_acc), hip.ptr(dv_acc), hip.ptr(dqkv),
            T, Hkv, D, G, row_len, H * D, D, (H + Hkv) * D, hip.BF16,
        ),
        "fin",
    )


ms = timed(fin)
gb = (2 * T * H * D * 4 + 2 * T * Hkv * D * 2) / 1e9
print(f"finalize   : {ms:6.3f} ms  {gb/ms*1e3:6.0f} GB/s ({gb/ms*1e3/PEAK*100:4.1f}% of peak)")

Hn = 2560
x = torch.randn(T, Hn, dtype=torch.bfloat16, device=dev).requires_grad_(True)
w = (torch.randn(Hn, dtype=torch.bfloat16, device=dev) * 0.1 + 1.0).requires_grad_(True)
r = torch.randn(T, Hn, dtype=torch.bfloat16, device=dev).requires_grad_(True)
y, s = Fx.fused_rmsnorm(x, w, 1e-5, residual=r)
dy = torch.randn_like(y)
ds = torch.randn_like(s)
g = torch.autograd.grad((y, s), (x, r, w), (dy, ds), retain_graph=True)


def nb():
    torch.autograd.grad((y, s), (x, r, w), (dy, ds), retain_graph=True)


ms = timed(nb)
gb = (5 * T * Hn * 2) / 1e9
print(f"norm_bwd   : {ms:6.3f} ms  {gb/ms*1e3:6.0f} GB/s ({gb/ms*1e3/PEAK*100:4.1f}% of peak)")
```

Measured before the change: 51970 tokens/s.

## Process two query heads per wave in flash-attention forward and dQ kernels

Adds a head-pair mode where each wave computes two query heads that share the same KV head (GQA/MQA). Each K/V tile staged into LDS and each K/V fragment read then feeds two heads' MFMAs. To fit the extra registers, the paired kernels use 4-wave workgroups (64 query rows) and adjusted launch bounds. Pairing is on by default when there is no dropout and the padded head dim is 64 or 96 (dQ only at 64), with a runtime toggle. The cost is higher register pressure, smaller query tiles and a larger grid, which may lower occupancy.

```diff
diff --git a/dolomite_engine_amd/csrc/attention.hip b/dolomite_engine_amd/csrc/attention.hip
--- a/dolomite_engine_amd/csrc/attention.hip
+++ b/dolomite_engine_amd/csrc/attention.hip
@@ -1,5 +1,7 @@
 
 #include "common.h"
+
+#include <atomic>
 
 typedef __bf16 bf16x8 __attribute__((ext_vector_type(8)));
 typedef float f32x4 __attribute__((ext_vector_type(4)));
@@ -166,8 +168,22 @@
 }
 
 
-template <int DPAD, bool DROPOUT>
-__global__ void __launch_bounds__(512, 4) fa_fwd_kernel(
+#ifndef DOLOMITE_FA_PAIR_WAVES
+#define DOLOMITE_FA_PAIR_WAVES 4
+#endif
+constexpr int FA_PAIR_WAVES = DOLOMITE_FA_PAIR_WAVES;
+static_assert(FA_PAIR_WAVES == 8 || FA_PAIR_WAVES == 4, "paired workgroup: 8 or 4 waves");
+constexpr int fa_waves(int hpw) { return hpw == 1 ? 8 : FA_PAIR_WAVES; }
+constexpr int fa_min_waves_per_simd(int hpw, int nw, bool roomy = false) {
+    return hpw == 1 ? 4 : (nw == 8 || roomy ? 2 : 3);
+}
+constexpr int fa_stage_pieces(int dpad, int nw) { return nw == 8 ? 2 : (64 * dpad / 8 + nw * 64 - 1) / (nw * 64); }
+#define FA_EACH_HEAD(...)                     \
+    { constexpr int hp = 0; __VA_ARGS__ }     \
+    if constexpr (HPW > 1) { constexpr int hp = 1; __VA_ARGS__ }
+
+template <int DPAD, bool DROPOUT, int HPW = 1, int NW = 8>
+__global__ void __launch_bounds__(NW * 64, fa_min_waves_per_simd(HPW, NW, DPAD > 96)) fa_fwd_kernel(
     const __bf16* __restrict__ q, const __bf16* __restrict__ k, const __bf16* __restrict__ v,
     __bf16* __restrict__ o, float* __restrict__ lse,
     const int32_t* __restrict__ seq_begin, const int32_t* __restrict__ seq_end,
@@ -178,14 +194,18 @@
     constexpr int KCH = DPAD / 32;
     constexpr int DCH = DPAD / 16;
     constexpr int SK = FaKvLds<DPAD>::S;
+    constexpr int NT = NW * 64;
+    constexpr int QROWS = NW * 16;
+    static_assert(HPW == 1 || (HPW == 2 && !DROPOUT), "head pairs: no dropout form");
 
     int tile_id = blockIdx.x, b = blockIdx.y, h = blockIdx.z;
     xcd_remap_tile_bh(tile_id, b, h);
+    h *= HPW;
     const int s0 = __builtin_amdgcn_readfirstlane(seq_begin[b]);
     const int L = __builtin_amdgcn_readfirstlane(seq_end[b]) - s0;
-    const int ntile_seq = (L + 127) / 128;
+    const int ntile_seq = (L + QROWS - 1) / QROWS;
     if (tile_id >= ntile_seq) return;
-    const int qs = (ntile_seq - 1 - tile_id) * 128;
+    const int qs = (ntile_seq - 1 - tile_id) * QROWS;
 
     const int lane = threadIdx.x & 63;
     const int wave = threadIdx.x >> 6;
@@ -202,18 +222,20 @@
 
     const int qrow = qs + wave * 16 + lr;
     const bool qvalid = qrow < L;
-    bf16x8 qf[KCH];
-#pragma unroll
-    for (int kc = 0; kc < KCH; ++kc) {
-        int d0 = kc * 32 + lg * 8;
-        const __bf16* p = q + (int64_t)(s0 + (qvalid ? qrow : 0)) * q_ts + q_hoff + d0;
-        qf[kc] = load_bf16x8_guard(p, d0, D, qvalid);
-    }
-
-    float m_run = -INFINITY, l_run = 0.f;
-    f32x4 o_acc[DCH];
-#pragma unroll
-    for (int dc = 0; dc < DCH; ++dc) o_acc[dc] = {0.f, 0.f, 0.f, 0.f};
+    bf16x8 qf[HPW][KCH];
+    FA_EACH_HEAD(
+        _Pragma("unroll") for (int kc = 0; kc < KCH; ++kc) {
+            int d0 = kc * 32 + lg * 8;
+            const __bf16* p = q + (int64_t)(s0 + (qvalid ? qrow : 0)) * q_ts + q_hoff + hp * D + d0;
+            qf[hp][kc] = load_bf16x8_guard(p, d0, D, qvalid);
+        })
+
+    float m_run[HPW], l_run[HPW];
+    f32x4 o_acc[HPW][DCH];
+    FA_EACH_HEAD(
+        m_run[hp] = -INFINITY;
+        l_run[hp] = 0.f;
+        _Pragma("unroll") for (int dc = 0; dc < DCH; ++dc) o_acc[hp][dc] = {0.f, 0.f, 0.f, 0.f};)
 
     uint32_t drop_rw = 0;
     uint32_t drop_hw = 0;
@@ -225,11 +247,11 @@
     unsigned aV0, aV1;
     fa_tr16_perm_bases(Vlds, SK, lane, aV0, aV1);
 
-    const int kend = min(L, qs + 128);
+    const int kend = min(L, qs + QROWS);
     const int ntiles = (kend + 63) / 64;
 
     if (D < DPAD) {
-        for (int pidx = threadIdx.x; pidx < 64 * (DPAD - D) / 8; pidx += 512) {
+        for (int pidx = threadIdx.x; pidx < 64 * (DPAD - D) / 8; pidx += NT) {
             int key = pidx / ((DPAD - D) / 8);
             int d0 = D + (pidx % ((DPAD - D) / 8)) * 8;
             bf16x8 z = {};
@@ -238,11 +260,12 @@
         }
     }
 
-    int st_koff[2], st_voff[2];
-    int st_klds[2], st_vlds[2];
-#pragma unroll
-    for (int j = 0; j < 2; ++j) {
-        int pidx = (int)threadIdx.x + j * 512;
+    constexpr int NST = fa_stage_pieces(DPAD, NW);
+    int st_koff[NST], st_voff[NST];
+    int st_klds[NST], st_vlds[NST];
+#pragma unroll
+    for (int j = 0; j < NST; ++j) {
+        int pidx = (int)threadIdx.x + j * NT;
         int pp = pidx < 64 * D / 8 ? pidx : 0;
         int key = pp / (D / 8);
         int d0 = (pp % (D / 8)) * 8;
@@ -252,7 +275,9 @@
         st_vlds[j] = key * SK + d0;
     }
 
-    if (__builtin_amdgcn_readfirstlane(threadIdx.x) >= 256) __builtin_amdgcn_s_setprio(1);
+    if constexpr (NW == 8) {
+        if (__builtin_amdgcn_readfirstlane(threadIdx.x) >= 256) __builtin_amdgcn_s_setprio(1);
+    }
 
     constexpr int PIECES = 64 * DPAD / 8;
 
@@ -260,14 +285,14 @@
         if (ks_ + 64 <= kend) {
             const int64_t disp = (int64_t)(s0 + ks_);
 #pragma unroll
-            for (int j = 0; j < 2; ++j) {
-                if ((int)threadIdx.x + j * 512 < 64 * D / 8) {
+            for (int j = 0; j < NST; ++j) {
+                if ((int)threadIdx.x + j * NT < 64 * D / 8) {
                     *(bf16x8*)&Kw[st_klds[j]] = *(const bf16x8*)(k + disp * k_ts + st_koff[j]);
                     *(bf16x8*)&Vw[st_vlds[j]] = *(const bf16x8*)(v + disp * v_ts + st_voff[j]);
                 }
             }
         } else {
-            for (int pidx = threadIdx.x; pidx < PIECES; pidx += 512) {
+            for (int pidx = threadIdx.x; pidx < PIECES; pidx += NT) {
                 int key = pidx / (DPAD / 8);
                 int d0 = (pidx % (DPAD / 8)) * 8;
                 bool kv_valid = (ks_ + key) < kend;
@@ -282,14 +307,14 @@
     const float scale2 = scale * DOL_LOG2E;
 
     auto compute_tile = [&](const __bf16* Kb, unsigned aV0c, unsigned aV1c, int ks) {
-        f32x4 sc[4];
+        f32x4 sc[HPW][4];
 #pragma unroll
         for (int cb = 0; cb < 4; ++cb) {
-            sc[cb] = {0.f, 0.f, 0.f, 0.f};
+            FA_EACH_HEAD(sc[hp][cb] = {0.f, 0.f, 0.f, 0.f};)
 #pragma unroll
             for (int kc = 0; kc < KCH; ++kc) {
                 bf16x8 kf = *(const bf16x8*)&Kb[(cb * 16 + lr) * SK + kc * 32 + lg * 8];
-                sc[cb] = MFMA16(kf, qf[kc], sc[cb]);
+                FA_EACH_HEAD(sc[hp][cb] = MFMA16(kf, qf[hp][kc], sc[hp][cb]);)
             }
         }
 
@@ -301,40 +326,38 @@
 #pragma unroll
                 for (int x = 0; x < 4; ++x) {
                     const int kpos = ks + cb * 16 + lg * 4 + x;
-                    if (kpos > qrow || kpos >= kend || qrow >= L) sc[cb][x] = -INFINITY;
+                    const bool masked = kpos > qrow || kpos >= kend || qrow >= L;
+                    FA_EACH_HEAD(if (masked) sc[hp][cb][x] = -INFINITY;)
                 }
             }
         }
-        float mx[4];
-#pragma unroll
-        for (int cb = 0; cb < 4; ++cb)
-            mx[cb] = fmaxf(fmaxf(sc[cb][0], sc[cb][1]), fmaxf(sc[cb][2], sc[cb][3]));
-        const float rowmax = qgroup_reduce_max(fmaxf(fmaxf(mx[0], mx[1]), fmaxf(mx[2], mx[3])));
-        float mnew = fmaxf(m_run, rowmax * scale2);
-        if (mnew == -INFINITY) mnew = 0.f;
-        const float alpha = exp2f(m_run - mnew);
-        m_run = mnew;
-
-        bf16x8 pf[2];
-        float rsum = 0.f;
-#pragma unroll
-        for (int cb = 0; cb < 4; ++cb) {
-            u32x4 cw = {};
-            if constexpr (DROPOUT) cw = *(const u32x4*)&Cw[cb * 16 + lg * 4];
-#pragma unroll
-            for (int x = 0; x < 4; ++x) {
-                const float e = exp2f(fmaf(sc[cb][x], scale2, -mnew));
-                float ek = e;
-                if constexpr (DROPOUT) ek = drop_keep_words(drop_rw, cw[x], drop_thr) ? e : 0.f;
-                pf[cb >> 1][(cb & 1) * 4 + x] = (__bf16)ek;
-                rsum += e;
+        bf16x8 pf[HPW][2];
+        FA_EACH_HEAD(
+            float mx[4];
+            _Pragma("unroll") for (int cb = 0; cb < 4; ++cb)
+                mx[cb] = fmaxf(fmaxf(sc[hp][cb][0], sc[hp][cb][1]), fmaxf(sc[hp][cb][2], sc[hp][cb][3]));
+            const float rowmax = qgroup_reduce_max(fmaxf(fmaxf(mx[0], mx[1]), fmaxf(mx[2], mx[3])));
+            float mnew = fmaxf(m_run[hp], rowmax * scale2);
+            if (mnew == -INFINITY) mnew = 0.f;
+            const float alpha = exp2f(m_run[hp] - mnew);
+            m_run[hp] = mnew;
+
+            float rsum = 0.f;
+            _Pragma("unroll") for (int cb = 0; cb < 4; ++cb) {
+                u32x4 cw = {};
+                if constexpr (DROPOUT) cw = *(const u32x4*)&Cw[cb * 16 + lg * 4];
+                _Pragma("unroll") for (int x = 0; x < 4; ++x) {
+                    const float e = exp2f(fmaf(sc[hp][cb][x], scale2, -mnew));
+                    float ek = e;
+                    if constexpr (DROPOUT) ek = drop_keep_words(drop_rw, cw[x], drop_thr) ? e : 0.f;
+                    pf[hp][cb >> 1][(cb & 1) * 4 + x] = (__bf16)ek;
+                    rsum += e;
+                }
             }
-        }
-        l_run = l_run * alpha + rsum;
-        if (!__all(alpha == 1.0f)) {
-#pragma unroll
-            for (int dc = 0; dc < DCH; ++dc) o_acc[dc] *= alpha;
-        }
+            l_run[hp] = l_run[hp] * alpha + rsum;
+            if (!__all(alpha == 1.0f)) {
+                _Pragma("unroll") for (int dc = 0; dc < DCH; ++dc) o_acc[hp][dc] *= alpha;
+            })
 
         {
             __builtin_amdgcn_sched_barrier(0);
@@ -353,7 +376,8 @@
         } else {                                                                                        \
             lgkm_wait2<0>(vlo[(i) % 3], vhi[(i) % 3]);                                                  \
         }                                                                                               \
-        o_acc[dc_] = MFMA16(tr16_join8(vlo[(i) % 3], vhi[(i) % 3]), pf[kc2_], o_acc[dc_]);              \
+        const bf16x8 vf_ = tr16_join8(vlo[(i) % 3], vhi[(i) % 3]);                                      \
+        FA_EACH_HEAD(o_acc[hp][dc_] = MFMA16(vf_, pf[hp][kc2_], o_acc[hp][dc_]);)                       \
     }
             FWD_PV_STEP(0) FWD_PV_STEP(1) FWD_PV_STEP(2) FWD_PV_STEP(3)
             FWD_PV_STEP(4) FWD_PV_STEP(5) FWD_PV_STEP(6) FWD_PV_STEP(7)
@@ -375,20 +399,19 @@
         __syncthreads();
     }
 
-    const float l_row = qgroup_reduce_sum(l_run);
-    float inv_l = (l_row > 0.f) ? 1.f / l_row : 0.f;
-    if constexpr (DROPOUT) inv_l *= drop_rp;
-    if (lg == 0 && qvalid)
-        lse[(int64_t)h * T_total + s0 + qrow] = (m_run + log2f(l_row)) * DOL_LN2;
-    __bf16* orow = o + (int64_t)(s0 + (qvalid ? qrow : 0)) * o_ts + (int64_t)h * D;
-#pragma unroll
-    for (int dc = 0; dc < DCH; ++dc) {
-        const int d0 = dc * 16 + lg * 4;
-        bf16x4 ov;
-#pragma unroll
-        for (int x = 0; x < 4; ++x) ov[x] = (__bf16)(o_acc[dc][x] * inv_l);
-        if (qvalid && d0 < D) *(bf16x4*)&orow[d0] = ov;
-    }
+    FA_EACH_HEAD(
+        const float l_row = qgroup_reduce_sum(l_run[hp]);
+        float inv_l = (l_row > 0.f) ? 1.f / l_row : 0.f;
+        if constexpr (DROPOUT) inv_l *= drop_rp;
+        if (lg == 0 && qvalid)
+            lse[(int64_t)(h + hp) * T_total + s0 + qrow] = (m_run[hp] + log2f(l_row)) * DOL_LN2;
+        __bf16* orow = o + (int64_t)(s0 + (qvalid ? qrow : 0)) * o_ts + (int64_t)(h + hp) * D;
+        _Pragma("unroll") for (int dc = 0; dc < DCH; ++dc) {
+            const int d0 = dc * 16 + lg * 4;
+            bf16x4 ov;
+            _Pragma("unroll") for (int x = 0; x < 4; ++x) ov[x] = (__bf16)(o_acc[hp][dc][x] * inv_l);
+            if (qvalid && d0 < D) *(bf16x4*)&orow[d0] = ov;
+        })
 }
 
 struct FaProblem {
@@ -431,17 +454,54 @@
     return p.p_drop > 0.f ? by_dpad(std::true_type{}) : by_dpad(std::false_type{});
 }
 
-static dim3 fa_grid(const FaProblem& p) { return dim3((p.max_seqlen + 127) / 128, p.batch, p.H); }
-
-template <int DPAD, bool DROPOUT>
-static int launch_fa_fwd(const FaProblem& p) {
-    hipLaunchKernelGGL((fa_fwd_kernel<DPAD, DROPOUT>), fa_grid(p), dim3(512), FaKvLds<DPAD>::bytes(DROPOUT),
+static dim3 fa_grid(const FaProblem& p, int hpw = 1, int nw = 8) {
+    return dim3((p.max_seqlen + nw * 16 - 1) / (nw * 16), p.batch, p.H / hpw);
+}
+
+
+constexpr bool fa_pair_fwd_enabled(int dpad) { return dpad == 64 || dpad == 96; }
+constexpr bool fa_pair_dq_enabled(int dpad) { return dpad == 64; }
+
+static std::atomic<int> fa_head_pairing_mode{1};
+
+extern "C" int dolomite_fa_head_pairing(int mode) {
+    if (mode == 0 || mode == 1) fa_head_pairing_mode.store(mode);
+    return fa_head_pairing_mode.load();
+}
+
+extern "C" int dolomite_fa_heads_per_wave(int H, int Hkv, int D, int G, float p_drop) {
+    (void)Hkv;
+    if (fa_head_pairing_mode.load() != 1) return 1;
+    if (G <= 0 || G % 2 != 0 || H % 2 != 0) return 1;
+    if (p_drop != 0.f) return 1;
+    if (D <= 0 || D > 128) return 1;
+    const int dpad = D <= 32 ? 32 : D <= 64 ? 64 : D <= 96 ? 96 : 128;
+    return fa_pair_fwd_enabled(dpad) ? 2 : 1;
+}
+
+static bool fa_use_head_pairs(const FaProblem& p) {
+    return dolomite_fa_heads_per_wave(p.H, p.Hkv, p.D, p.G, p.p_drop) == 2;
+}
+
+template <int DPAD, bool DROPOUT, int HPW>
+static int launch_fa_fwd_hpw(const FaProblem& p) {
+    constexpr int NW = fa_waves(HPW);
+    hipLaunchKernelGGL((fa_fwd_kernel<DPAD, DROPOUT, HPW, NW>), fa_grid(p, HPW, NW), dim3(NW * 64),
+                       FaKvLds<DPAD>::bytes(DROPOUT),
                        (hipStream_t)p.stream, (const __bf16*)p.q, (const __bf16*)p.k, (const __bf16*)p.v,
                        (__bf16*)p.o, p.lse, p.seq_begin, p.seq_end, p.H, p.Hkv, p.D, p.G,
                        p.q_ts, p.q_gs, p.k_ts, p.k_hs, p.v_ts, p.v_hs, (int64_t)p.H * p.D, p.T, p.scale,
                        (uint32_t)p.seed, (uint32_t)(p.seed >> 32), drop_threshold(p.p_drop),
                        1.f / (1.f - p.p_drop));
     return dol_last_error();
+}
+
+template <int DPAD, bool DROPOUT>
+static int launch_fa_fwd(const FaProblem& p) {
+    if constexpr (!DROPOUT && fa_pair_fwd_enabled(DPAD)) {
+        if (fa_use_head_pairs(p)) return launch_fa_fwd_hpw<DPAD, false, 2>(p);
+    }
+    return launch_fa_fwd_hpw<DPAD, DROPOUT, 1>(p);
 }
 
 static int fa_spans_fwd_dispatch(const FaProblem& p) {
@@ -817,8 +877,8 @@
     }
 }
 
-template <int DPAD, bool DROPOUT>
-__global__ void __launch_bounds__(512, (DROPOUT && DPAD > 96) ? 2 : 4) fa_bwd_dq_kernel(
+template <int DPAD, bool DROPOUT, int HPW = 1, int NW = 8>
+__global__ void __launch_bounds__(NW * 64, (DROPOUT && DPAD > 96) ? 2 : fa_min_waves_per_simd(HPW, NW, DPAD > 64)) fa_bwd_dq_kernel(
     const __bf16* __restrict__ q, const __bf16* __restrict__ k, const __bf16* __restrict__ v,
     const __bf16* __restrict__ dout, const float* __restrict__ lse, const float* __restrict__ delta,
     __bf16* __restrict__ dqkv_q,
@@ -829,15 +889,19 @@
     uint32_t seed_lo, uint32_t seed_hi, uint32_t drop_thr, float drop_rp) {
     constexpr int KCH = DPAD / 32;
     constexpr int DCH = DPAD / 16;
+    constexpr int NT = NW * 64;
+    constexpr int QROWS = NW * 16;
+    static_assert(HPW == 1 || (HPW == 2 && !DROPOUT), "head pairs: no dropout form");
 
     int tile_id = blockIdx.x, b = blockIdx.y, h = blockIdx.z;
     xcd_remap_tile_bh(tile_id, b, h);
+    h *= HPW;
     const int kvh = h / G;
     const int s0 = __builtin_amdgcn_readfirstlane(seq_begin[b]);
     const int L = __builtin_amdgcn_readfirstlane(seq_end[b]) - s0;
-    const int ntile_seq = (L + 127) / 128;
+    const int ntile_seq = (L + QROWS - 1) / QROWS;
     if (tile_id >= ntile_seq) return;
-    const int qs = (ntile_seq - 1 - tile_id) * 128;
+    const int qs = (ntile_seq - 1 - tile_id) * QROWS;
 
     const int lane = threadIdx.x & 63;
     const int wave = threadIdx.x >> 6;
@@ -858,23 +922,23 @@
 
     const int qrow = qs + wave * 16 + lr;
     const bool qvalid = qrow < L;
-    bf16x8 qfr[KCH], dfr[KCH];
-#pragma unroll
-    for (int kc = 0; kc < KCH; ++kc) {
-        int d0 = kc * 32 + lg * 8;
-        const __bf16* qp = q + (int64_t)(s0 + (qvalid ? qrow : 0)) * q_ts + q_hoff + d0;
-        qfr[kc] = load_bf16x8_guard(qp, d0, D, qvalid);
-        const __bf16* dp = dout + (int64_t)(s0 + (qvalid ? qrow : 0)) * do_ts + do_hoff + d0;
-        dfr[kc] = load_bf16x8_guard(dp, d0, D, qvalid);
-    }
-
-    const float lsev = qvalid ? lse[(int64_t)h * T_total + s0 + qrow] * DOL_LOG2E : 0.f;
-    const float delv = qvalid ? delta[(int64_t)h * T_total + s0 + qrow] : 0.f;
+    bf16x8 qfr[HPW][KCH], dfr[HPW][KCH];
+    float lsev[HPW], delv[HPW];
+    f32x4 dq[HPW][DCH];
+    FA_EACH_HEAD(
+        _Pragma("unroll") for (int kc = 0; kc < KCH; ++kc) {
+            int d0 = kc * 32 + lg * 8;
+            const __bf16* qp = q + (int64_t)(s0 + (qvalid ? qrow : 0)) * q_ts + q_hoff + hp * D + d0;
+            qfr[hp][kc] = load_bf16x8_guard(qp, d0, D, qvalid);
+            const __bf16* dp = dout + (int64_t)(s0 + (qvalid ? qrow : 0)) * do_ts + do_hoff + hp * D + d0;
+            dfr[hp][kc] = load_bf16x8_guard(dp, d0, D, qvalid);
+        })
+    FA_EACH_HEAD(
+        lsev[hp] = qvalid ? lse[(int64_t)(h + hp) * T_total + s0 + qrow] * DOL_LOG2E : 0.f;
+        delv[hp] = qvalid ? delta[(int64_t)(h + hp) * T_total + s0 + qrow] : 0.f;)
     const float scale2 = scale * DOL_LOG2E;
-
-    f32x4 dq[DCH];
-#pragma unroll
-    for (int dc = 0; dc < DCH; ++dc) dq[dc] = {0.f, 0.f, 0.f, 0.f};
+    FA_EACH_HEAD(
+        _Pragma("unroll") for (int dc = 0; dc < DCH; ++dc) dq[hp][dc] = {0.f, 0.f, 0.f, 0.f};)
 
     uint32_t drop_rw = 0;
     uint32_t drop_hw = 0;
@@ -884,7 +948,7 @@
     }
 
     if (D < DPAD) {
-        for (int pidx = threadIdx.x; pidx < 64 * (DPAD - D) / 8; pidx += 512) {
+        for (int pidx = threadIdx.x; pidx < 64 * (DPAD - D) / 8; pidx += NT) {
             int key = pidx / ((DPAD - D) / 8);
             int d0 = D + (pidx % ((DPAD - D) / 8)) * 8;
             bf16x8 z = {};
@@ -893,11 +957,12 @@
         }
     }
 
-    int st_koff[2], st_voff[2];
-    int st_klds[2], st_vlds[2];
-#pragma unroll
-    for (int j = 0; j < 2; ++j) {
-        int pidx = (int)threadIdx.x + j * 512;
+    constexpr int NST = fa_stage_pieces(DPAD, NW);
+    int st_koff[NST], st_voff[NST];
+    int st_klds[NST], st_vlds[NST];
+#pragma unroll
+    for (int j = 0; j < NST; ++j) {
+        int pidx = (int)threadIdx.x + j * NT;
         int pp = pidx < 64 * D / 8 ? pidx : 0;
         int key = pp / (D / 8);
         int d0 = (pp % (D / 8)) * 8;
@@ -907,10 +972,12 @@
         st_vlds[j] = key * SQ + d0;
     }
 
-    const int kend_total = min(L, qs + 128);
+    const int kend_total = min(L, qs + QROWS);
     const int nkt = (kend_total + 63) / 64;
 
-    if (__builtin_amdgcn_readfirstlane(threadIdx.x) >= 256) __builtin_amdgcn_s_setprio(1);
+    if constexpr (NW == 8) {
+        if (__builtin_amdgcn_readfirstlane(threadIdx.x) >= 256) __builtin_amdgcn_s_setprio(1);
+    }
 
     for (int kt = 0; kt < nkt; ++kt) {
         const int ks = kt * 64;
@@ -920,14 +987,14 @@
             if (ks + 64 <= kend_total) {
                 const int64_t disp = (int64_t)(s0 + ks);
 #pragma unroll
-                for (int j = 0; j < 2; ++j) {
-                    if ((int)threadIdx.x + j * 512 < 64 * D / 8) {
+                for (int j = 0; j < NST; ++j) {
+                    if ((int)threadIdx.x + j * NT < 64 * D / 8) {
                         *(bf16x8*)&Klds[st_klds[j]] = *(const bf16x8*)(k + disp * k_ts + st_koff[j]);
                         *(bf16x8*)&Vlds[st_vlds[j]] = *(const bf16x8*)(v + disp * v_ts + st_voff[j]);
                     }
                 }
             } else {
-                for (int pidx = threadIdx.x; pidx < pieces; pidx += 512) {
+                for (int pidx = threadIdx.x; pidx < pieces; pidx += NT) {
                     int key = pidx / (DPAD / 8);
                     int d0 = (pidx % (DPAD / 8)) * 8;
                     bool valid = (ks + key) < kend_total;
@@ -945,41 +1012,42 @@
         __syncthreads();
 
         const bool full_tile = (ks + 64 <= qs + wave * 16 + 1) && (ks + 64 <= kend_total) && (qs + wave * 16 + 16 <= L);
-        bf16x8 dsf[2];
+        bf16x8 dsf[HPW][2];
 #pragma unroll
         for (int cb = 0; cb < 4; ++cb) {
-            f32x4 sc = {0.f, 0.f, 0.f, 0.f};
-            f32x4 dp = {0.f, 0.f, 0.f, 0.f};
+            f32x4 sc[HPW], dp[HPW];
+            FA_EACH_HEAD(sc[hp] = {0.f, 0.f, 0.f, 0.f}; dp[hp] = {0.f, 0.f, 0.f, 0.f};)
 #pragma unroll
             for (int kc = 0; kc < KCH; ++kc) {
                 int d0 = kc * 32 + lg * 8;
                 bf16x8 kb = *(const bf16x8*)&Klds[(cb * 16 + lr) * SQ + d0];
-                sc = MFMA16(kb, qfr[kc], sc);
+                FA_EACH_HEAD(sc[hp] = MFMA16(kb, qfr[hp][kc], sc[hp]);)
                 bf16x8 vb = *(const bf16x8*)&Vlds[(cb * 16 + lr) * SQ + d0];
-                dp = MFMA16(vb, dfr[kc], dp);
+                FA_EACH_HEAD(dp[hp] = MFMA16(vb, dfr[hp][kc], dp[hp]);)
             }
             u32x4 cw = {};
             if constexpr (DROPOUT) cw = *(const u32x4*)&Cw[cb * 16 + lg * 4];
             if (__builtin_amdgcn_readfirstlane(full_tile ? 1 : 0)) {
-#pragma unroll
-                for (int x = 0; x < 4; ++x) {
-                    float pv = exp2f(fmaf(sc[x], scale2, -lsev));
-                    float dpm = dp[x];
-                    if constexpr (DROPOUT)
-                        dpm = drop_keep_words(drop_rw, cw[x], drop_thr) ? dp[x] * drop_rp : 0.f;
-                    dsf[cb >> 1][(cb & 1) * 4 + x] = (__bf16)(pv * (dpm - delv) * scale);
-                }
+                FA_EACH_HEAD(
+                    _Pragma("unroll") for (int x = 0; x < 4; ++x) {
+                        float pv = exp2f(fmaf(sc[hp][x], scale2, -lsev[hp]));
+                        float dpm = dp[hp][x];
+                        if constexpr (DROPOUT)
+                            dpm = drop_keep_words(drop_rw, cw[x], drop_thr) ? dp[hp][x] * drop_rp : 0.f;
+                        dsf[hp][cb >> 1][(cb & 1) * 4 + x] = (__bf16)(pv * (dpm - delv[hp]) * scale);
+                    })
             } else {
 #pragma unroll
                 for (int x = 0; x < 4; ++x) {
                     const int kpos = ks + cb * 16 + lg * 4 + x;
                     bool ok = qvalid && kpos < kend_total && kpos <= qrow;
-                    float pv = ok ? exp2f(fmaf(sc[x], scale2, -lsev)) : 0.f;
-                    float dpm = dp[x];
-                    if constexpr (DROPOUT)
-                        dpm = drop_keep_words(drop_rw, cw[x], drop_thr) ? dp[x] * drop_rp : 0.f;
-                    float ds = ok ? pv * (dpm - delv) * scale : 0.f;
-                    dsf[cb >> 1][(cb & 1) * 4 + x] = (__bf16)ds;
+                    FA_EACH_HEAD(
+                        float pv = ok ? exp2f(fmaf(sc[hp][x], scale2, -lsev[hp])) : 0.f;
+                        float dpm = dp[hp][x];
+                        if constexpr (DROPOUT)
+                            dpm = drop_keep_words(drop_rw, cw[x], drop_thr) ? dp[hp][x] * drop_rp : 0.f;
+                        float ds = ok ? pv * (dpm - delv[hp]) * scale : 0.f;
+                        dsf[hp][cb >> 1][(cb & 1) * 4 + x] = (__bf16)ds;)
                 }
             }
         }
@@ -1004,7 +1072,8 @@
         } else {                                                                                        \
             lgkm_wait2<0>(klo[(i) % 4], khi[(i) % 4]);                                                  \
         }                                                                                               \
-        dq[dc_] = MFMA16(tr16_join8(klo[(i) % 4], khi[(i) % 4]), dsf[kc2_], dq[dc_]);                   \
+        const bf16x8 kf_ = tr16_join8(klo[(i) % 4], khi[(i) % 4]);                                      \
+        FA_EACH_HEAD(dq[hp][dc_] = MFMA16(kf_, dsf[hp][kc2_], dq[hp][dc_]);)                            \
     }
             DQ_STEP(0) DQ_STEP(1) DQ_STEP(2) DQ_STEP(3)
             DQ_STEP(4) DQ_STEP(5) DQ_STEP(6) DQ_STEP(7)
@@ -1015,16 +1084,16 @@
         }
     }
 
-    __bf16* dqrow = dqkv_q + (int64_t)(s0 + (qvalid ? qrow : 0)) * q_ts + q_hoff;
-#pragma unroll
-    for (int dc = 0; dc < DCH; ++dc) {
-        const int d0 = dc * 16 + lg * 4;
-        bf16x4 dv;
-#pragma unroll
-        for (int x = 0; x < 4; ++x) dv[x] = (__bf16)dq[dc][x];
-        if (qvalid && d0 < D) *(bf16x4*)&dqrow[d0] = dv;
-    }
-}
+    FA_EACH_HEAD(
+        __bf16* dqrow = dqkv_q + (int64_t)(s0 + (qvalid ? qrow : 0)) * q_ts + q_hoff + hp * D;
+        _Pragma("unroll") for (int dc = 0; dc < DCH; ++dc) {
+            const int d0 = dc * 16 + lg * 4;
+            bf16x4 dv;
+            _Pragma("unroll") for (int x = 0; x < 4; ++x) dv[x] = (__bf16)dq[hp][dc][x];
+            if (qvalid && d0 < D) *(bf16x4*)&dqrow[d0] = dv;
+        })
+}
+#undef FA_EACH_HEAD
 
 template <int DPAD, bool DROPOUT>
 static int launch_fa_bwd(const FaProblem& p) {
@@ -1041,6 +1110,17 @@
                        p.T, p.scale, seed_lo, seed_hi, thr, rp);
     int err = dol_last_error();
     if (err) return err;
+    if constexpr (!DROPOUT && fa_pair_fwd_enabled(DPAD) && fa_pair_dq_enabled(DPAD)) {
+        if (fa_use_head_pairs(p)) {
+            constexpr int NW = fa_waves(2);
+            hipLaunchKernelGGL((fa_bwd_dq_kernel<DPAD, false, 2, NW>), fa_grid(p, 2, NW), dim3(NW * 64),
+                               FaKvLds<DPAD>::bytes(false), stream,
+                               q, k, v, dout, p.lse, p.delta, (__bf16*)p.dqkv_q, p.seq_begin, p.seq_end,
+                               p.H, p.Hkv, p.D, p.G, p.q_ts, p.q_gs, p.k_ts, p.k_hs, p.v_ts, p.v_hs, p.do_ts,
+                               p.T, p.scale, seed_lo, seed_hi, thr, rp);
+            return dol_last_error();
+        }
+    }
     hipLaunchKernelGGL((fa_bwd_dq_kernel<DPAD, DROPOUT>), grid, block, FaKvLds<DPAD>::bytes(DROPOUT), stream,
                        q, k, v, dout, p.lse, p.delta, (__bf16*)p.dqkv_q, p.seq_begin, p.seq_end,
                        p.H, p.Hkv, p.D, p.G, p.q_ts, p.q_gs, p.k_ts, p.k_hs, p.v_ts, p.v_hs, p.do_ts,
diff --git a/dolomite_engine_amd/ops/hip.py b/dolomite_engine_amd/ops/hip.py
--- a/dolomite_engine_amd/ops/hip.py
+++ b/dolomite_engine_amd/ops/hip.py
@@ -32,6 +32,8 @@
     "dolomite_fa_bwd_preprocess": ([_p, _p, _p, _p, _i64, _i32, _i32, _i64, _i64, _i32], _i32),
     "dolomite_fa_zero_gap_rows": ([_p, _p, _i64, _p, _p, _i32, _i64], _i32),
     "dolomite_fa_dropout_mask_probe": ([_p, _p, _u64, _f32, _i32, _i64, _i32, _i64, _i32], _i32),
+    "dolomite_fa_head_pairing": ([_i32], _i32),
+    "dolomite_fa_heads_per_wave": ([_i32, _i32, _i32, _i32, _f32], _i32),
     "dolomite_kv_cache_append": (
         [_p, _p, _p, _p, _p, _p, _p, _i32, _i32, _i32, _i32, _i32,
          _i64, _i64, _i64, _i64, _i64, _i64, _i64, _i32],
diff --git a/include/dolomite_hip.h b/include/dolomite_hip.h
--- a/include/dolomite_hip.h
+++ b/include/dolomite_hip.h
@@ -125,6 +125,9 @@
                               const int32_t* seq_begin, const int32_t* seq_end,
                               int batch, int64_t T);
 
+int dolomite_fa_head_pairing(int mode);
+int dolomite_fa_heads_per_wave(int H, int Hkv, int D, int G, float p_drop);
+
 int dolomite_fa_dropout_mask_probe(dolomite_stream_t stream, uint8_t* out,
                                    uint64_t seed, float p_drop, int H,
                                    int64_t tq0, int nq, int64_t tk0, int nk);
diff --git a/tools_kernel_micro.py b/tools_kernel_micro.py
--- a/tools_kernel_micro.py
+++ b/tools_kernel_micro.py
@@ -109,8 +109,84 @@
         assert out.shape == (B, S + 128)
 
 
+def headpair_case(rounds=4, warm=3, n=12):
+    from pathlib import Path
+
+    from dolomite_engine_amd.ops.functional import QKVLayout
+
+    if "--lib" in sys.argv:
+        hip._SO_PATH = Path(sys.argv[sys.argv.index("--lib") + 1]).resolve()
+    lib = hip.lib()
+    print(f"library: {hip.so_path()}")
+    shapes = [
+        ("3b bench shape", "mqa", 32, 1, 80, 16, 4096),
+        ("350m          ", "mqa", 16, 1, 64, 64, 2048),
+        ("llama8b       ", "gqa", 32, 8, 128, 2, 8192),
+    ]
+    for name, head_type, H, Hkv, D, B, S in shapes:
+        lo = QKVLayout.make(H, Hkv, D, head_type)
+        T = B * S
+        scale = 1.0 / math.sqrt(D)
+        qkv = (torch.randn(T, lo.row_len, device=dev) * 0.5).to(torch.bfloat16)
+        do = (torch.randn(T, H * D, device=dev) * 0.5).to(torch.bfloat16)
+        cu = torch.arange(0, T + 1, S, dtype=torch.int32, device=dev)
+        delta = torch.empty(H, T, dtype=torch.float32, device=dev)
+
+        def alloc():
+            return dict(
+                o=torch.empty(T, H * D, dtype=torch.bfloat16, device=dev),
+                lse=torch.empty(H, T, dtype=torch.float32, device=dev),
+                dqkv=torch.zeros(T, lo.row_len, dtype=torch.bfloat16, device=dev),
+                dk=torch.empty(T, H, D, dtype=torch.float32, device=dev),
+                dv=torch.empty(T, H, D, dtype=torch.float32, device=dev),
+            )
+
+        def fwd(r):
+            hip.check(lib.dolomite_fa_varlen_fwd(
+                hip.stream(), *lo.operands(qkv), hip.ptr(r["o"]), hip.ptr(r["lse"]), hip.ptr(cu), B, S, T,
+                H, Hkv, D, lo.G, *lo.strides(), scale, hip.BF16), "fwd")
+
+        def bwd(r):
+            hip.check(lib.dolomite_fa_varlen_bwd(
+                hip.stream(), *lo.operands(qkv), hip.ptr(do), hip.ptr(r["lse"]), hip.ptr(delta),
+                hip.ptr(r["dqkv"]), hip.ptr(r["dk"]), hip.ptr(r["dv"]), hip.ptr(cu), B, S, T,
+                H, Hkv, D, lo.G, *lo.strides(), H * D, scale, hip.BF16), "bwd")
+
+        res = {0: alloc(), 1: alloc()}
+        hpw = {}
+        for mode in (0, 1):
+            assert lib.dolomite_fa_head_pairing(mode) == mode
+            hpw[mode] = lib.dolomite_fa_heads_per_wave(H, Hkv, D, lo.G, 0.0)
+            fwd(res[mode])
+            if mode == 0:
+                hip.check(lib.dolomite_fa_bwd_preprocess(
+                    hip.stream(), hip.ptr(res[0]["o"]), hip.ptr(do), hip.ptr(delta), T, H, D, H * D, H * D,
+                    hip.BF16), "pre")
+            bwd(res[mode])
+        torch.cuda.synchronize()
+        print(f"--- {name}: {head_type} H={H} Hkv={Hkv} D={D} T={T} ({B} x {S}); "
+              f"heads per wave: off {hpw[0]}, on {hpw[1]} ---")
+        same = {k: torch.equal(res[0][k], res[1][k]) for k in res[0]}
+        print("bitwise equal off vs on: " + "  ".join(f"{k}={v}" for k, v in same.items()))
+        for rnd in range(rounds):
+            line = []
+            for mode in (0, 1):
+                lib.dolomite_fa_head_pairing(mode)
+                f_med, f_min, _ = timed_median(lambda: fwd(res[mode]), n=n, warm=warm)
+                b_med, b_min, _ = timed_median(lambda: bwd(res[mode]), n=n, warm=warm)
+                line.append((f_med, f_min, b_med, b_min))
+            (f0, f0m, b0, b0m), (f1, f1m, b1, b1m) = line
+            print(f"round {rnd}: fwd off {f0:.3f} (min {f0m:.3f})  on {f1:.3f} (min {f1m:.3f})  {100 * (f0 / f1 - 1):+5.1f}%"
+                  f" | bwd off {b0:.3f} (min {b0m:.3f})  on {b1:.3f} (min {b1m:.3f})  {100 * (b0 / b1 - 1):+5.1f}%   [ms]")
+        lib.dolomite_fa_head_pairing(1)
+        del res, qkv, do, delta
+
+
 if len(sys.argv) > 1 and sys.argv[1] == "decode":
     decode_case()
+    sys.exit(0)
+if len(sys.argv) > 1 and sys.argv[1] == "headpair":
+    headpair_case(rounds=int(sys.argv[sys.argv.index("--rounds") + 1]) if "--rounds" in sys.argv else 4)
     sys.exit(0)
 
 o = torch.randn(T, H * D, dtype=torch.bfloat16, device=dev)
```

Result: no change. 52480 tokens/s (median of 6 runs) (+1.0%).
